# libmir/mir-optim

Measured on AMD Instinct MI355X. Metric: LM iterations/sec, higher is better.
Workload: dtype f64

## Files before the change

include/mir_optim_amd.h:

```cpp
#ifndef MIR_OPTIM_AMD_H
#define MIR_OPTIM_AMD_H

#include <stddef.h>
#include <stdint.h>

#ifdef __cplusplus
extern "C" {
#endif


typedef enum mir_least_squares_status {
    mir_ls_maxIterations = -1,
    mir_ls_furtherImprovement = 0,
    mir_ls_xConverged = 1,
    mir_ls_gConverged = 2,
    mir_ls_fConverged = 3,
    mir_ls_badBounds = -32,
    mir_ls_badGuess = -31,
    mir_ls_badMinStepQuality = -30,
    mir_ls_badGoodStepQuality = -29,
    mir_ls_badStepQuality = -28,
    mir_ls_badLambdaParams = -27,
    mir_ls_numericError = -26
} mir_least_squares_status;
// ... 29 lines not shown
    uint32_t maxIterations, maxAge;
    float jacobianEpsilon, absTolerance, relTolerance, gradTolerance, maxGoodResidual, maxStep,
          maxLambda, minLambda, minStepQuality, goodStepQuality, lambdaIncrease, lambdaDecrease;
    mir_box_qp_settings_s qpSettings;
} mir_least_squares_settings_s;

typedef struct mir_least_squares_result_d {
    int32_t status;
    uint32_t iterations, fCalls, gCalls;
    double residual;
    double lambda;
} mir_least_squares_result_d;
typedef struct mir_least_squares_result_s {
    int32_t status;
    uint32_t iterations, fCalls, gCalls;
    float residual, lambda;
} mir_least_squares_result_s;

typedef struct mir_slice_d { size_t length; double* ptr; } mir_slice_d;
typedef struct mir_slice_s { size_t length; float* ptr; } mir_slice_s;
typedef struct mir_slice_i { size_t length; int32_t* ptr; } mir_slice_i;

typedef void (*mir_least_squares_function_d)(void* context, size_t m, size_t n, const double* x, double* y);
typedef void (*mir_least_squares_jacobian_d)(void* context, size_t m, size_t n, const double* x, double* J);
typedef void (*mir_least_squares_function_s)(void* context, size_t m, size_t n, const float* x, float* y);
typedef void (*mir_least_squares_jacobian_s)(void* context, size_t m, size_t n, const float* x, float* J);

typedef struct mir_least_squares_task { void* context; void* function; } mir_least_squares_task;
typedef void (*mir_least_squares_task_function)(mir_least_squares_task task, uint32_t totalThreads,
                                                uint32_t threadId, uint32_t i);
typedef void (*mir_least_squares_thread_manager)(void* context, uint32_t count,
                                                 mir_least_squares_task taskContext,
                                                 mir_least_squares_task_function task);

size_t mir_least_squares_work_length(size_t m, size_t n);
size_t mir_least_squares_iwork_length(size_t m, size_t n);
size_t mir_box_qp_work_length(size_t n);
size_t mir_box_qp_iwork_length(size_t n);
size_t mir_box_qp_iwork_length_ilp64(size_t n);
size_t mir_least_squares_iwork_length_ilp64(size_t m, size_t n);
const char* mir_least_squares_status_string(mir_least_squares_status st);
void mir_least_squares_init_d(mir_least_squares_settings_d* settings);
void mir_least_squares_init_s(mir_least_squares_settings_s* settings);
void mir_least_squares_reset_d(mir_least_squares_settings_d* settings);
void mir_least_squares_reset_s(mir_least_squares_settings_s* settings);

mir_least_squares_result_d mir_optimize_least_squares_d(
    const mir_least_squares_settings_d* settings, size_t m, size_t n,
    double* x, const double* l, const double* u,
    mir_slice_d work, mir_slice_i iwork,
    void* fContext, mir_least_squares_function_d f,
    void* gContext, mir_least_squares_jacobian_d g,
    void* tmContext, mir_least_squares_thread_manager tm);

mir_least_squares_result_s mir_optimize_least_squares_s(
    const mir_least_squares_settings_s* settings, size_t m, size_t n,
    float* x, const float* l, const float* u,
    mir_slice_s work, mir_slice_i iwork,
    void* fContext, mir_least_squares_function_s f,
    void* gContext, mir_least_squares_jacobian_s g,
    void* tmContext, mir_least_squares_thread_manager tm);


typedef struct mir_lsq_comm mir_lsq_comm;
typedef struct mir_lsq_workspace mir_lsq_workspace;

typedef void (*mir_lsq_batched_function_d)(void* context, size_t m, size_t n, size_t p, const double* X, double* Y);
typedef void (*mir_lsq_batched_function_s)(void* context, size_t m, size_t n, size_t p, const float* X, float* Y);
enum {
    MIR_LSQ_DEVICE_CALLBACKS = 1u,
    MIR_LSQ_TIME_KERNELS = 2u,
    MIR_LSQ_FD_BASE_POINT = 4u
};

enum {
    MIR_LSQ_VARIANT_BROYDEN_REWRITE = 1u << 0,
    MIR_LSQ_VARIANT_FD_SEPARATE_FILL = 1u << 1,
    MIR_LSQ_VARIANT_NO_SPECULATION = 1u << 4,
    MIR_LSQ_VARIANT_NO_NULL_SKIP = 1u << 5,
    MIR_LSQ_VARIANT_SOLVE_BOUNDED = 1u << 6,
    MIR_LSQ_VARIANT_SOLVE_GENERIC = 1u << 10,
    MIR_LSQ_VARIANT_SOLVE_ONE_WORKGROUP = 1u << 11,
    MIR_LSQ_VARIANT_NO_FD_BASE_POINT = 1u << 14,
    MIR_LSQ_VARIANT_FD_HOST_COLUMNS = 1u << 13,
    MIR_LSQ_VARIANT_NO_PIPELINE = 1u << 22,
    MIR_LSQ_VARIANT_DEBUG_HELPERS_ABSENT = 1u << 12,
    MIR_LSQ_VARIANT_DEBUG_SOLVE = 1u << 7,
    MIR_LSQ_VARIANT_HOST_PROFILE = 1u << 8,
    MIR_LSQ_VARIANT_LR_CAP_SHIFT = 16
};

typedef struct mir_lsq_stats {
    uint64_t passes, accepted, rejected, step_guard_rejects;
    uint64_t jacobian_full, jacobian_broyden;
    uint64_t jtj_launches;
    uint64_t jtj_broyden_launches;
    double jtj_ms;
    double jtj_broyden_ms;
    double solve_ms;
    uint64_t solve_launches;
    double fd_ms;
    double total_ms;
    uint64_t qp_active_set_passes;
    uint64_t broyden_lr_columns;
    double jtj_fd_ms;
    uint64_t jtj_fd_launches;
    uint64_t elided_evaluations;
    uint64_t allreduce_calls[3];
    uint64_t allreduce_elems[3];
    uint64_t broyden_flushes;
    uint64_t jtj_resyncs;
    double fd_callback_ms;
    uint64_t fd_callback_calls, fd_callback_points;
    double trial_callback_ms;
    uint64_t trial_callback_calls, trial_callback_points;
    uint64_t library_launches;
    uint64_t round_launches[3];
    uint64_t rounds[3];
    double fd_host_wall_ms, fd_host_f_ms;
    uint64_t fd_host_columns;
    double host_f_ms;
    uint64_t host_f_calls;
    uint64_t fused_rounds;
    uint64_t fused_passes;
    uint64_t coop_timeouts;
} mir_lsq_stats;

typedef struct mir_lsq_trace_record {
    int32_t event;
    uint32_t iterations;
    double lambda, residual, trial_residual, dx_dot;
} mir_lsq_trace_record;
typedef struct mir_lsq_trace {
    mir_lsq_trace_record* records;
    uint64_t capacity;
    uint64_t count;
} mir_lsq_trace;

typedef struct mir_lsq_gpu_options {
    uint32_t struct_size;
    uint32_t flags;
    void* stream;
    mir_lsq_comm* comm;
    mir_lsq_workspace* workspace;
    void* fbContext;
    void* fb;
    uint32_t fd_batch;
    uint32_t variant;
    mir_lsq_stats* stats;
    mir_lsq_trace* trace;
    void* fbRowMajor;
    void* fbRowMajorDiff;
    uint32_t stats_size;
    uint32_t reserved0;
} mir_lsq_gpu_options;

mir_least_squares_result_d mir_optimize_least_squares_gpu_d(
    const mir_least_squares_settings_d* settings, size_t m, size_t n,
    double* x, const double* l, const double* u, const mir_lsq_gpu_options* options,
    void* fContext, mir_least_squares_function_d f,
    void* gContext, mir_least_squares_jacobian_d g,
    void* tmContext, mir_least_squares_thread_manager tm);
mir_least_squares_result_s mir_optimize_least_squares_gpu_s(
    const mir_least_squares_settings_s* settings, size_t m, size_t n,
    float* x, const float* l, const float* u, const mir_lsq_gpu_options* options,
    void* fContext, mir_least_squares_function_s f,
// ... 112 lines not shown
                                              const double* t, size_t t_stride, const double* data,
                                              mir_least_squares_result_d* results, const mir_lsq_batched_options* options,
                                              const mir_lsq_batched_extras* extras);
int mir_lsq_batched16_kernel_ex_d(const mir_least_squares_settings_d* settings, size_t count, size_t m, int model,
                                  double* x, const double* lower, const double* upper,
                                  const double* t, size_t t_stride, const double* data,
                                  mir_least_squares_result_d* results, const mir_lsq_batched_options* options,
                                  const mir_lsq_batched_extras* extras);
int mir_lsq_batched16_covariance_d(const mir_least_squares_settings_d* settings, size_t count, size_t m, int model,
                                   const double* x, const double* lower, const double* upper,
                                   const double* t, size_t t_stride, const double* data,
                                   const mir_least_squares_result_d* results, const mir_lsq_batched_options* options,
                                   const mir_lsq_batched_extras* extras);
int mir_lsq_batched16_jtj_d(size_t count, size_t m, size_t n, const double* J, const double* y, double* JJ, double* Jy, void* stream);

enum { MIR_LSQ_RESIDENT_NO_NULL_SKIP = 1u,
       MIR_LSQ_RESIDENT_UNBOUNDED = 2u,
       MIR_LSQ_RESIDENT_NO_LOOKAHEAD = 4u,
       MIR_LSQ_RESIDENT_DEBUG_DROP_WORKGROUP = 16u,
       MIR_LSQ_RESIDENT_ANALYTIC_JACOBIAN = 32u,
       MIR_LSQ_RESIDENT_NO_STAMPS = 8u           };
typedef struct mir_lsq_resident_stats {
    uint64_t rounds, passes, accepted, rejected, step_guard_rejects, jacobian_full, jacobian_broyden, qp_active_set_passes,
        elided_evaluations;
    uint64_t t_total, t_stage, t_worker, t_group, t_total_wait, t_solver, t_solve_body, t_cmd_wait;
    uint64_t t_w_eval, t_w_fd, t_w_prod;
    uint64_t t_w_mma;
    uint64_t lookahead_rejections;
    uint64_t t_look;
    uint64_t t_unpack, t_publish;
    uint32_t abort_code, grid, rows, groups;
} mir_lsq_resident_stats;
typedef struct mir_lsq_resident_options {
    uint32_t struct_size;
    uint32_t variant;
    void* stream;
    void* workspace;
    size_t workspace_bytes;
    mir_lsq_trace_record* trace_records;
    uint32_t trace_capacity;
    uint32_t max_workgroups;
    uint32_t* trace_count;
    mir_lsq_resident_stats* stats;
} mir_lsq_resident_options;

int mir_lsq_batched_posvx_s(size_t count, size_t n, const float* P, const float* rhs, float* x, int* info, void* stream);
int mir_lsq_batched_posvx_d(size_t count, size_t n, const double* P, const double* rhs, double* x, int* info, void* stream);
int mir_lsq_batched_posvx16_s(size_t count, size_t n, const float* P, const float* rhs, float* x, int* info, void* stream);
int mir_lsq_batched_posvx16_d(size_t count, size_t n, const double* P, const double* rhs, double* x, int* info, void* stream);

int mir_lsq_jtj_d(size_t m, size_t n, double* J, const double* y, const double* y_old, const double* dx,
                  int broyden, double* JJ, double* Jy, void* stream, float* kernel_ms);
int mir_lsq_jtj_s(size_t m, size_t n, float* J, const float* y, const float* y_old, const float* dx,
                  int broyden, float* JJ, float* Jy, void* stream, float* kernel_ms);
int mir_lsq_fd_jtj_d(size_t m, size_t n, const double* Yrm, const double* twh, const double* y, double* J,
                     double* JJ, double* Jy, void* stream, float* kernel_ms);
int mir_lsq_fd_diff_jtj_d(size_t m, size_t n, const double* Drm, const double* twh, const double* y, double* J,
                          double* JJ, double* Jy, void* stream, float* kernel_ms);
int mir_lsq_jtj_plan(size_t elem_size, size_t m, size_t n, int num_cu, int op, int aligned16, size_t out[10]);

enum { MIR_LSQ_LM_SOLVE_CHECK_GRAD = 1u, MIR_LSQ_LM_SOLVE_LAMBDA_FROM_STATE = 2u, MIR_LSQ_LM_SOLVE_FORCE_BOUNDED = 4u,
       MIR_LSQ_LM_SOLVE_GENERIC = 8u, MIR_LSQ_LM_SOLVE_ONE_WORKGROUP = 16u };
#define MIR_LSQ_LM_SOLVE_SENTINEL (-123456.0)
typedef struct { double lambda, new_dx_dot, predicted, trial_xnorm; int32_t qp_status, qp_iterations, flags, reserved; } mir_lsq_lm_solve_record_d;
typedef struct { float  lambda, new_dx_dot, predicted, trial_xnorm; int32_t qp_status, qp_iterations, flags, reserved; } mir_lsq_lm_solve_record_s;
int mir_lsq_lm_solve_d(const mir_least_squares_settings_d* settings, size_t n, double* JJ, double* Jy, double* x, double* lower,
                       double* upper, int ks, const double* lam, double state_lambda, unsigned mode, mir_lsq_lm_solve_record_d* rec,
                       double* dx, double* trial, double* jy_inf, int info[6]);
int mir_lsq_lm_solve_s(const mir_least_squares_settings_s* settings, size_t n, float* JJ, float* Jy, float* x, float* lower,
                       float* upper, int ks, const float* lam, float state_lambda, unsigned mode, mir_lsq_lm_solve_record_s* rec,
                       float* dx, float* trial, float* jy_inf, int info[6]);
int mir_lsq_lm_solve_class(size_t elem_size, size_t n, int bounded, int generic, int diagnostic, int out[3]);

int mir_lsq_lr_pass_d(size_t m, size_t n, int k, const double* J, double* U, double* D, const double* dx, const double* dx_dot,
                      const double* y, int count, const double* y_old, double* JJ, double* Jy, const mir_lsq_lm_solve_record_d* spec,
                      double absTolerance, double relTolerance, double* partials, double* reduced, double* sums, double* jy_inf,
                      int info[6]);
int mir_lsq_lr_pass_s(size_t m, size_t n, int k, const float* J, float* U, float* D, const float* dx, const float* dx_dot,
                      const float* y, int count, const float* y_old, float* JJ, float* Jy, const mir_lsq_lm_solve_record_s* spec,
                      float absTolerance, float relTolerance, float* partials, float* reduced, float* sums, float* jy_inf,
                      int info[6]);
int mir_lsq_lr_flush_d(size_t m, size_t n, int k, double* J, const double* U, const double* D, int info[2]);
int mir_lsq_lr_flush_s(size_t m, size_t n, int k, float* J, const float* U, const float* D, int info[2]);
int mir_lsq_lr_class(size_t elem_size, size_t n, int aligned, int out[2]);
int mir_lsq_lr_blocks(size_t m, int num_cu);

typedef struct {
    double lambda, mu, residual, trial_residual, dx_dot, new_dx_dot, predicted, trial_xnorm, jy_inf, improvement, rho, pad0;
    int32_t qp_status, qp_iterations, flags, decision; uint32_t iterations; int32_t accepted_k;
    uint32_t consumed, fcalls, rejects, guards, qp_active, null_tail, seq, coop_rescued; int32_t spec_ok;
} mir_lsq_lm_state_d;
typedef struct {
    float lambda, mu, residual, trial_residual, dx_dot, new_dx_dot, predicted, trial_xnorm, jy_inf, improvement, rho, pad0;
    int32_t qp_status, qp_iterations, flags, decision; uint32_t iterations; int32_t accepted_k;
    uint32_t consumed, fcalls, rejects, guards, qp_active, null_tail, seq, coop_rescued; int32_t spec_ok;
} mir_lsq_lm_state_s;
enum { MIR_LSQ_DECIDE_CHECK_GRAD = 1u, MIR_LSQ_DECIDE_LAMBDA_FROM_STATE = 2u, MIR_LSQ_DECIDE_SPEC_STATIC = 4u, MIR_LSQ_DECIDE_MIRROR = 8u };
int mir_lsq_decide_d(const mir_least_squares_settings_d* settings, size_t n, int ks, unsigned mode, uint32_t maxIterations, uint32_t seq,
                     mir_lsq_lm_state_d* state, mir_lsq_lm_solve_record_d* rec, double* sums, double* x, double* trial, double* dx_chain,
                     double* dx_acc, double* partials, int nparts, int pstride, mir_lsq_lm_state_d* host_state, double* host_x, int info[2]);
int mir_lsq_decide_s(const mir_least_squares_settings_s* settings, size_t n, int ks, unsigned mode, uint32_t maxIterations, uint32_t seq,
                     mir_lsq_lm_state_s* state, mir_lsq_lm_solve_record_s* rec, float* sums, float* x, float* trial, float* dx_chain,
                     float* dx_acc, float* partials, int nparts, int pstride, mir_lsq_lm_state_s* host_state, float* host_x, int info[2]);
int mir_lsq_fd_points_d(size_t n, const double* x, const double* lower, const double* upper, double eps, int with_base, double* X,
                        double* twh, double* twh_host, int info[2]);
int mir_lsq_fd_points_s(size_t n, const float* x, const float* lower, const float* upper, float eps, int with_base, float* X,
                        float* twh, float* twh_host, int info[2]);
int mir_lsq_fd_fill_d(size_t m, size_t n, size_t ldy, int j0, int pc, const double* Y, const double* twh, double* J, int col, int info[2]);
int mir_lsq_fd_fill_s(size_t m, size_t n, size_t ldy, int j0, int pc, const float* Y, const float* twh, float* J, int col, int info[2]);
int mir_lsq_entry_state_d(size_t m, const double* v, uint32_t seq, double* partials, double* sum, mir_lsq_lm_state_d* state,
                          mir_lsq_lm_state_d* host_state, double* partials2, double* sums2, mir_lsq_lm_state_d* st2, int info[3]);
int mir_lsq_entry_state_s(size_t m, const float* v, uint32_t seq, float* partials, float* sum, mir_lsq_lm_state_s* state,
                          mir_lsq_lm_state_s* host_state, float* partials2, float* sums2, mir_lsq_lm_state_s* st2, int info[3]);
int mir_lsq_sumsq_blocks(size_t m);
int mir_lsq_unpack_grad_d(size_t n, const double* packed, mir_lsq_lm_state_d* state, double* JJ, double* Jy, int info[2]);
int mir_lsq_unpack_grad_s(size_t n, const float* packed, mir_lsq_lm_state_s* state, float* JJ, float* Jy, int info[2]);

enum { MIR_LSQ_COVARIANCE_ABSOLUTE_SIGMA = 1u };
int mir_lsq_covariance_gpu_d(const mir_least_squares_settings_d* settings, size_t m, size_t n,
    const double* x, const double* l, const double* u, const mir_lsq_gpu_options* options,
    void* fContext, mir_least_squares_function_d f, void* gContext, mir_least_squares_jacobian_d g,
    void* tmContext, mir_least_squares_thread_manager tm,
    uint32_t flags, double* cov, double* residual_out, int* info);
int mir_lsq_covariance_gpu_s(const mir_least_squares_settings_s* settings, size_t m, size_t n,
    const float* x, const float* l, const float* u, const mir_lsq_gpu_options* options,
    void* fContext, mir_least_squares_function_s f, void* gContext, mir_least_squares_jacobian_s g,
    void* tmContext, mir_least_squares_thread_manager tm,
    uint32_t flags, float* cov, float* residual_out, int* info);
int mir_lsq_spd_inverse_d(size_t n, const double* P, const unsigned char* fixed, double* X, int* info, void* stream);
int mir_lsq_spd_inverse_s(size_t n, const float*  P, const unsigned char* fixed, float*  X, int* info, void* stream);
size_t mir_lsq_spd_inverse_work_bytes(size_t n, size_t elem_size);
int mir_lsq_spd_inverse_work_d(size_t n, const double* P, const unsigned char* fixed, double* X, int* info, void* work,
                               size_t work_bytes, void* stream);
int mir_lsq_spd_inverse_work_s(size_t n, const float* P, const unsigned char* fixed, float* X, int* info, void* work,
                               size_t work_bytes, void* stream);

mir_lsq_workspace* mir_lsq_workspace_create(size_t m, size_t n, size_t elem_size);
void mir_lsq_workspace_destroy(mir_lsq_workspace* ws);

int mir_lsq_rccl_unique_id(void* out_128_bytes);
mir_lsq_comm* mir_lsq_comm_create_rccl(int nranks, int rank, const void* unique_id_128_bytes);
typedef void (*mir_lsq_allreduce_fn)(void* ctx, double* device_buf, size_t count, void* stream);
mir_lsq_comm* mir_lsq_comm_create_callback(int nranks, int rank, mir_lsq_allreduce_fn fn, void* ctx);
int mir_lsq_comm_create_local_group(int nranks, mir_lsq_comm** out_comms);
void mir_lsq_comm_destroy(mir_lsq_comm* comm);
int mir_lsq_comm_record(mir_lsq_comm* comm, double* host_buf, size_t capacity);
size_t mir_lsq_comm_recorded(const mir_lsq_comm* comm);
mir_lsq_comm* mir_lsq_comm_create_replay(int nranks, int rank, const double* totals_host, size_t len, mir_lsq_comm* inner);
int mir_lsq_comm_replay_rewind(mir_lsq_comm* comm);
int mir_lsq_comm_replay_set_delay(mir_lsq_comm* comm, unsigned microseconds);
int mir_lsq_comm_ranks(const mir_lsq_comm* comm);
int mir_lsq_comm_describe(const mir_lsq_comm* comm, char* buf, size_t len);
int mir_lsq_comm_allreduce_d(mir_lsq_comm* comm, double* buf, size_t count, void* stream);
int mir_lsq_comm_allreduce_s(mir_lsq_comm* comm, float* buf, size_t count, void* stream);

int mir_lsq_device_count(void);
void* mir_lsq_device_malloc(size_t bytes);
void mir_lsq_device_free(void* p);
int mir_lsq_memcpy_h2d(void* dst_device, const void* src_host, size_t bytes, void* stream);
int mir_lsq_memcpy_d2h(void* dst_host, const void* src_device, size_t bytes, void* stream);
int mir_lsq_memcpy_d2d(void* dst_device, const void* src_device, size_t bytes, void* stream);

int mir_lsq_selftest_reductions(int rounds, int mismatches[4]);
void* mir_lsq_stream_create(void);
void mir_lsq_stream_destroy(void* stream);
int mir_lsq_stream_synchronize(void* stream);
// ... 43 lines not shown
```

mir_optim_amd/api.py:

```python
import ctypes as C
import enum
import os
import types

import numpy as np

from . import build as _build

__all__ = [
    "LeastSquaresStatus", "BoxQPStatus", "LeastSquaresSettings", "LeastSquaresResult", "BoxQPSettings",
    "LeastSquaresException", "optimize", "optimizeLeastSquares", "solveBoxQP", "leastSquaresStatusString",
    "mir_least_squares_work_length", "mir_least_squares_iwork_length", "mir_box_qp_work_length",
    "mir_box_qp_iwork_length", "GpuOptions", "Stats", "lib", "workloads_lib", "device_count",
    "DeviceBuffer", "Stream", "jtj", "fd_jtj", "DEVICE_CALLBACKS", "TIME_KERNELS", "optimizeLeastSquaresBatched", "batchedPosvx", "BATCHED_NO_LADDER", "BATCHED_DEVICE_BOUNDS",
    "solveBoxQPBatched", "BOX_QP_UNCONSTRAINED_SOLUTION",
    "MODEL_EXP_DECAY", "MODEL_EXP3_AFFINE", "MODEL_EXP_DECAY_PAD8", "MODEL16_EXP_HARM16", "MODEL16_GAUSS3_AFFINE", "batched16JtJ", "optimizeLeastSquaresBatched16", "ResultS", "Trace", "TraceRecord", "Spline", "FitSplineResult", "fitSpline",
    "fit_spline_residuals", "variant_lr_cap",
    "VARIANT_BROYDEN_REWRITE", "VARIANT_FD_SEPARATE_FILL", "VARIANT_NO_SPECULATION", "VARIANT_NO_NULL_SKIP",
    "VARIANT_SOLVE_BOUNDED", "VARIANT_DEBUG_SOLVE", "VARIANT_HOST_PROFILE", "VARIANT_SOLVE_GENERIC", "VARIANT_SOLVE_ONE_WORKGROUP", "VARIANT_DEBUG_HELPERS_ABSENT", "VARIANT_FD_HOST_COLUMNS",
    "VARIANT_NO_PIPELINE", "FD_BASE_POINT", "VARIANT_NO_FD_BASE_POINT", "BatchedOptions", "BatchedExtras", "BATCHED_ABSOLUTE_SIGMA", "BATCHED_BOUNDS_PER_PROBLEM",
    "covariance", "spdInverse", "COVARIANCE_ABSOLUTE_SIGMA",
    "fitSplineGpu", "splineEvalGpu", "fit_spline_eval_gpu", "fit_spline_eval_host", "fit_spline_factor",
    "lmSolve", "lm_solve_class",
    "lrPass", "lrFlush", "lr_class", "lr_blocks", "lr_len",
    "lm_state_dtype", "lmDecide", "fdPoints", "fdFill", "entryState", "sumsq_blocks", "unpackGrad",
]

MODEL_EXP_DECAY = 0
MODEL_EXP3_AFFINE = 1
MODEL_EXP_DECAY_PAD8 = 2
MODEL16_EXP_HARM16 = 16
MODEL16_GAUSS3_AFFINE = 17
_MODELS16 = (MODEL16_EXP_HARM16, MODEL16_GAUSS3_AFFINE)

DEVICE_CALLBACKS = 1
TIME_KERNELS = 2
FD_BASE_POINT = 4

VARIANT_BROYDEN_REWRITE = 1 << 0
VARIANT_FD_SEPARATE_FILL = 1 << 1
VARIANT_NO_SPECULATION = 1 << 4
VARIANT_NO_NULL_SKIP = 1 << 5
VARIANT_SOLVE_BOUNDED = 1 << 6
VARIANT_DEBUG_SOLVE = 1 << 7
VARIANT_HOST_PROFILE = 1 << 8
VARIANT_SOLVE_GENERIC = 1 << 10
VARIANT_SOLVE_ONE_WORKGROUP = 1 << 11
VARIANT_DEBUG_HELPERS_ABSENT = 1 << 12
VARIANT_FD_HOST_COLUMNS = 1 << 13
VARIANT_NO_FD_BASE_POINT = 1 << 14
VARIANT_NO_PIPELINE = 1 << 22


def variant_lr_cap(k):
    return (int(k) & 31) << 16


class LeastSquaresStatus(enum.IntEnum):
    maxIterations = -1
    furtherImprovement = 0
    xConverged = 1
    gConverged = 2
    fConverged = 3
    badBounds = -32
    badGuess = -31
    badMinStepQuality = -30
    badGoodStepQuality = -29
    badStepQuality = -28
    badLambdaParams = -27
    numericError = -26


class BoxQPStatus(enum.IntEnum):
    solved = 0
    numericError = 1
    maxIterations = 2


class LeastSquaresException(Exception):

    def __init__(self, status, result=None):
        self.status = LeastSquaresStatus(status)
        self.result = result
        super().__init__("mir-optim Least Squares: " + leastSquaresStatusString(status))


class _QPd(C.Structure):
    _fields_ = [("relTolerance", C.c_double), ("absTolerance", C.c_double), ("maxIterations", C.c_uint32)]


class _QPs(C.Structure):
    _fields_ = [("relTolerance", C.c_float), ("absTolerance", C.c_float), ("maxIterations", C.c_uint32)]


_FIELDS = ["jacobianEpsilon", "absTolerance", "relTolerance", "gradTolerance", "maxGoodResidual", "maxStep",
           "maxLambda", "minLambda", "minStepQuality", "goodStepQuality", "lambdaIncrease", "lambdaDecrease"]


class _Sd(C.Structure):
    _fields_ = ([("maxIterations", C.c_uint32), ("maxAge", C.c_uint32)] + [(k, C.c_double) for k in _FIELDS]
                + [("qpSettings", _QPd)])


class _Ss(C.Structure):
    _fields_ = ([("maxIterations", C.c_uint32), ("maxAge", C.c_uint32)] + [(k, C.c_float) for k in _FIELDS]
                + [("qpSettings", _QPs)])


class _Rd(C.Structure):
    _fields_ = [("status", C.c_int32), ("iterations", C.c_uint32), ("fCalls", C.c_uint32), ("gCalls", C.c_uint32),
                ("residual", C.c_double), ("lambda_", C.c_double)]


class _Rs(C.Structure):
    _fields_ = [("status", C.c_int32), ("iterations", C.c_uint32), ("fCalls", C.c_uint32), ("gCalls", C.c_uint32),
                ("residual", C.c_float), ("lambda_", C.c_float)]


ResultS = _Rs


class _SliceD(C.Structure):
    _fields_ = [("length", C.c_size_t), ("ptr", C.c_void_p)]


class _Task(C.Structure):
    _fields_ = [("context", C.c_void_p), ("function", C.c_void_p)]


class Stats(C.Structure):
    _fields_ = [("passes", C.c_uint64), ("accepted", C.c_uint64), ("rejected", C.c_uint64),
                ("step_guard_rejects", C.c_uint64), ("jacobian_full", C.c_uint64), ("jacobian_broyden", C.c_uint64),
                ("jtj_launches", C.c_uint64), ("jtj_broyden_launches", C.c_uint64), ("jtj_ms", C.c_double),
# ... 96 lines not shown

def lib():
    global _lib
    if _lib is None:
        L = _load(_build.SOLVER_LIB)
        sz = C.c_size_t
        for name in ("mir_least_squares_work_length", "mir_least_squares_iwork_length"):
            getattr(L, name).restype = sz
            getattr(L, name).argtypes = [sz, sz]
        for name in ("mir_box_qp_work_length", "mir_box_qp_iwork_length"):
            getattr(L, name).restype = sz
            getattr(L, name).argtypes = [sz]
        L.mir_box_qp_iwork_length_ilp64.restype = sz
        L.mir_box_qp_iwork_length_ilp64.argtypes = [sz]
        L.mir_least_squares_iwork_length_ilp64.restype = sz
        L.mir_least_squares_iwork_length_ilp64.argtypes = [sz, sz]
        L.mir_least_squares_status_string.restype = C.c_char_p
        L.mir_least_squares_status_string.argtypes = [C.c_int]
        for suf, S, R in (("d", _Sd, _Rd), ("s", _Ss, _Rs)):
            getattr(L, "mir_least_squares_init_" + suf).argtypes = [C.POINTER(S)]
            getattr(L, "mir_least_squares_reset_" + suf).argtypes = [C.POINTER(S)]
            fn = getattr(L, "mir_optimize_least_squares_" + suf)
            fn.restype = R
            fn.argtypes = [C.POINTER(S), sz, sz, C.c_void_p, C.c_void_p, C.c_void_p, _SliceD, _SliceD,
                           C.c_void_p, C.c_void_p, C.c_void_p, C.c_void_p, C.c_void_p, C.c_void_p]
            fn = getattr(L, "mir_optimize_least_squares_gpu_" + suf)
            fn.restype = R
            fn.argtypes = [C.POINTER(S), sz, sz, C.c_void_p, C.c_void_p, C.c_void_p, C.POINTER(GpuOptions),
                           C.c_void_p, C.c_void_p, C.c_void_p, C.c_void_p, C.c_void_p, C.c_void_p]
            fn = getattr(L, "mir_solve_box_qp_gpu_" + suf)
            fn.restype = C.c_int
            fn.argtypes = [C.c_void_p, sz, C.c_void_p, C.c_void_p, C.c_void_p, C.c_void_p, C.c_void_p, C.c_int,
                           C.POINTER(C.c_int)]
            fn = getattr(L, "mir_lsq_jtj_" + suf)
            fn.restype = C.c_int
            fn.argtypes = [sz, sz, C.c_void_p, C.c_void_p, C.c_void_p, C.c_void_p, C.c_int, C.c_void_p, C.c_void_p,
                           C.c_void_p, C.POINTER(C.c_float)]
            fn = getattr(L, "mir_lsq_covariance_gpu_" + suf)
            fn.restype = C.c_int
            fn.argtypes = [C.POINTER(S), sz, sz, C.c_void_p, C.c_void_p, C.c_void_p, C.POINTER(GpuOptions),
                           C.c_void_p, C.c_void_p, C.c_void_p, C.c_void_p, C.c_void_p, C.c_void_p,
                           C.c_uint32, C.c_void_p, C.c_void_p, C.POINTER(C.c_int)]
            fn = getattr(L, "mir_lsq_spd_inverse_" + suf)
            fn.restype = C.c_int
            fn.argtypes = [sz, C.c_void_p, C.c_void_p, C.c_void_p, C.c_void_p, C.c_void_p]
            fn = getattr(L, "mir_lsq_spd_inverse_work_" + suf)
            fn.restype = C.c_int
            fn.argtypes = [sz, C.c_void_p, C.c_void_p, C.c_void_p, C.c_void_p, C.c_void_p, sz, C.c_void_p]
        L.mir_lsq_spd_inverse_work_bytes.restype = sz
        L.mir_lsq_spd_inverse_work_bytes.argtypes = [sz, sz]
        L.mir_lsq_comm_create_local_group.restype = C.c_int
        L.mir_lsq_comm_create_local_group.argtypes = [C.c_int, C.POINTER(C.c_void_p)]
        L.mir_lsq_fd_diff_jtj_d.restype = C.c_int
        L.mir_lsq_fd_diff_jtj_d.argtypes = [sz, sz, C.c_void_p, C.c_void_p, C.c_void_p, C.c_void_p, C.c_void_p, C.c_void_p,
                                            C.c_void_p, C.POINTER(C.c_float)]
        L.mir_lsq_fd_jtj_d.restype = C.c_int
        L.mir_lsq_fd_jtj_d.argtypes = [sz, sz, C.c_void_p, C.c_void_p, C.c_void_p, C.c_void_p, C.c_void_p, C.c_void_p,
                                       C.c_void_p, C.c_void_p]
        L.mir_optimize_least_squares_batched_s.restype = C.c_int
        L.mir_optimize_least_squares_batched_s.argtypes = [C.POINTER(_Ss), sz, sz, C.c_int, C.c_void_p, C.c_void_p, C.c_void_p,
                                                           C.c_void_p, sz, C.c_void_p, C.c_void_p, C.POINTER(BatchedOptions)]
        L.mir_lsq_batched_kernel_s.restype = C.c_int
        L.mir_lsq_batched_kernel_s.argtypes = [C.POINTER(_Ss), sz, sz, C.c_int, C.c_void_p, C.c_void_p, C.c_void_p,
                                               C.c_void_p, sz, C.c_void_p, C.c_void_p, C.POINTER(BatchedOptions)]
        L.mir_lsq_jtj_plan.restype = C.c_int
        L.mir_lsq_jtj_plan.argtypes = [sz, sz, sz, C.c_int, C.c_int, C.c_int, C.POINTER(sz * 10)]
        L.mir_lsq_selftest_reductions.restype = C.c_int
        L.mir_lsq_selftest_reductions.argtypes = [C.c_int, C.POINTER(C.c_int * 4)]
        for suf, S, ct in (("d", _Sd, C.c_double), ("s", _Ss, C.c_float)):
            fn = getattr(L, "mir_lsq_lm_solve_" + suf)
            fn.restype = C.c_int
            fn.argtypes = [C.POINTER(S), sz, C.c_void_p, C.c_void_p, C.c_void_p, C.c_void_p, C.c_void_p, C.c_int, C.c_void_p, ct,
                           C.c_uint, C.c_void_p, C.c_void_p, C.c_void_p, C.c_void_p, C.POINTER(C.c_int * 6)]
        L.mir_lsq_lm_solve_class.restype = C.c_int
        L.mir_lsq_lm_solve_class.argtypes = [sz, sz, C.c_int, C.c_int, C.c_int, C.POINTER(C.c_int * 3)]
        for suf, ct in (("d", C.c_double), ("s", C.c_float)):
            fn = getattr(L, "mir_lsq_lr_pass_" + suf)
            fn.restype = C.c_int
            fn.argtypes = [sz, sz, C.c_int] + [C.c_void_p] * 6 + [C.c_int] + [C.c_void_p] * 4 + [ct, ct] + [C.c_void_p] * 4 \
                + [C.POINTER(C.c_int * 6)]
            fn = getattr(L, "mir_lsq_lr_flush_" + suf)
            fn.restype = C.c_int
            fn.argtypes = [sz, sz, C.c_int, C.c_void_p, C.c_void_p, C.c_void_p, C.POINTER(C.c_int * 2)]
        L.mir_lsq_lr_class.restype = C.c_int
        L.mir_lsq_lr_class.argtypes = [sz, sz, C.c_int, C.POINTER(C.c_int * 2)]
        L.mir_lsq_lr_blocks.restype = C.c_int
        L.mir_lsq_lr_blocks.argtypes = [sz, C.c_int]
        vp, i2 = C.c_void_p, C.POINTER(C.c_int * 2)
        for suf, S, ct in (("d", _Sd, C.c_double), ("s", _Ss, C.c_float)):
            for name, args in (("decide", [C.POINTER(S), sz, C.c_int, C.c_uint, C.c_uint32, C.c_uint32] + [vp] * 8 + [C.c_int, C.c_int, vp, vp, i2]),
                               ("fd_points", [sz, vp, vp, vp, ct, C.c_int, vp, vp, vp, i2]),
                               ("fd_fill", [sz, sz, sz, C.c_int, C.c_int, vp, vp, vp, C.c_int, i2]),
                               ("entry_state", [sz, vp, C.c_uint32] + [vp] * 7 + [C.POINTER(C.c_int * 3)]),
                               ("unpack_grad", [sz, vp, vp, vp, vp, i2])):
                fn = getattr(L, "mir_lsq_%s_%s" % (name, suf))
                fn.restype, fn.argtypes = C.c_int, args
        L.mir_lsq_sumsq_blocks.restype = C.c_int
        L.mir_lsq_sumsq_blocks.argtypes = [sz]
        L.mir_lsq_batched_posvx_s.restype = C.c_int
        L.mir_lsq_batched_posvx_s.argtypes = [sz, sz, C.c_void_p, C.c_void_p, C.c_void_p, C.c_void_p, C.c_void_p]
        L.mir_optimize_least_squares_batched_d.restype = C.c_int
        L.mir_optimize_least_squares_batched_d.argtypes = [C.POINTER(_Sd), sz, sz, C.c_int, C.c_void_p, C.c_void_p, C.c_void_p,
                                                           C.c_void_p, sz, C.c_void_p, C.c_void_p, C.POINTER(BatchedOptions)]
        L.mir_lsq_batched_kernel_d.restype = C.c_int
        L.mir_lsq_batched_kernel_d.argtypes = [C.POINTER(_Sd), sz, sz, C.c_int, C.c_void_p, C.c_void_p, C.c_void_p,
                                               C.c_void_p, sz, C.c_void_p, C.c_void_p, C.POINTER(BatchedOptions)]
        L.mir_lsq_batched_posvx_d.restype = C.c_int
        L.mir_lsq_batched_posvx_d.argtypes = [sz, sz, C.c_void_p, C.c_void_p, C.c_void_p, C.c_void_p, C.c_void_p]
        for suf, S in (("s", _Ss), ("d", _Sd)):
            for name in ("mir_optimize_least_squares_batched_ex_", "mir_lsq_batched_kernel_ex_", "mir_lsq_batched_covariance_"):
                fn = getattr(L, name + suf)
                fn.restype = C.c_int
                fn.argtypes = [C.POINTER(S), sz, sz, C.c_int, C.c_void_p, C.c_void_p, C.c_void_p, C.c_void_p, sz, C.c_void_p,
                               C.c_void_p, C.POINTER(BatchedOptions), C.POINTER(BatchedExtras)]
        for name in ("mir_optimize_least_squares_batched16_d", "mir_lsq_batched16_kernel_d", "mir_optimize_least_squares_batched16_ex_d",
                     "mir_lsq_batched16_kernel_ex_d", "mir_lsq_batched16_covariance_d"):
            fn = getattr(L, name)
            fn.restype = C.c_int
            fn.argtypes = [C.POINTER(_Sd), sz, sz, C.c_int, C.c_void_p, C.c_void_p, C.c_void_p, C.c_void_p, sz, C.c_void_p,
                           C.c_void_p, C.POINTER(BatchedOptions), C.POINTER(BatchedExtras)]
        L.mir_lsq_batched16_jtj_d.restype = C.c_int
        L.mir_lsq_batched16_jtj_d.argtypes = [sz, sz, sz, C.c_void_p, C.c_void_p, C.c_void_p, C.c_void_p, C.c_void_p]
        for name in ("box_qp_s", "box_qp_d", "box_qp16_s", "box_qp16_d"):
            fn = getattr(L, "mir_lsq_batched_" + name)
            fn.restype = C.c_int
            fn.argtypes = [C.c_void_p, sz, sz, C.c_void_p, C.c_void_p, C.c_void_p, C.c_void_p, sz, C.c_void_p, C.c_void_p,
                           C.c_void_p, C.c_uint, C.c_void_p]
        for suf in ("s", "d"):
            fn = getattr(L, "mir_lsq_batched_posvx16_" + suf)
            fn.restype = C.c_int
            fn.argtypes = [sz, sz, C.c_void_p, C.c_void_p, C.c_void_p, C.c_void_p, C.c_void_p]
        L.mir_lsq_comm_describe.restype = C.c_int
        L.mir_lsq_comm_describe.argtypes = [C.c_void_p, C.c_char_p, C.c_size_t]
        L.mir_lsq_workspace_create.restype = C.c_void_p
        L.mir_lsq_workspace_create.argtypes = [sz, sz, sz]
        L.mir_lsq_workspace_destroy.argtypes = [C.c_void_p]
        L.mir_lsq_rccl_unique_id.restype = C.c_int
        L.mir_lsq_rccl_unique_id.argtypes = [C.c_void_p]
        L.mir_lsq_comm_create_rccl.restype = C.c_void_p
        L.mir_lsq_comm_create_rccl.argtypes = [C.c_int, C.c_int, C.c_void_p]
        L.mir_lsq_comm_create_callback.restype = C.c_void_p
        L.mir_lsq_comm_create_callback.argtypes = [C.c_int, C.c_int, ALLREDUCE_FN, C.c_void_p]
        L.mir_lsq_comm_destroy.argtypes = [C.c_void_p]
        L.mir_lsq_comm_record.restype = C.c_int
        L.mir_lsq_comm_record.argtypes = [C.c_void_p, C.c_void_p, sz]
        L.mir_lsq_comm_recorded.restype = sz
        L.mir_lsq_comm_recorded.argtypes = [C.c_void_p]
        L.mir_lsq_comm_create_replay.restype = C.c_void_p
        L.mir_lsq_comm_create_replay.argtypes = [C.c_int, C.c_int, C.c_void_p, sz, C.c_void_p]
        L.mir_lsq_comm_replay_rewind.restype = C.c_int
        L.mir_lsq_comm_replay_rewind.argtypes = [C.c_void_p]
        L.mir_lsq_comm_replay_set_delay.restype = C.c_int
        L.mir_lsq_comm_replay_set_delay.argtypes = [C.c_void_p, C.c_uint]
        L.mir_lsq_comm_ranks.restype = C.c_int
        L.mir_lsq_comm_ranks.argtypes = [C.c_void_p]
        for name in ("mir_lsq_comm_allreduce_d", "mir_lsq_comm_allreduce_s"):
            getattr(L, name).restype = C.c_int
            getattr(L, name).argtypes = [C.c_void_p, C.c_void_p, sz, C.c_void_p]
        L.mir_lsq_device_count.restype = C.c_int
        L.mir_lsq_device_malloc.restype = C.c_void_p
        L.mir_lsq_device_malloc.argtypes = [sz]
        L.mir_lsq_device_free.argtypes = [C.c_void_p]
        for name in ("mir_lsq_memcpy_h2d", "mir_lsq_memcpy_d2h", "mir_lsq_memcpy_d2d"):
            getattr(L, name).restype = C.c_int
            getattr(L, name).argtypes = [C.c_void_p, C.c_void_p, sz, C.c_void_p]
        L.mir_lsq_stream_create.restype = C.c_void_p
# ... 483 lines not shown
    fn = L.mir_solve_box_qp_gpu_d if dtype == np.float64 else L.mir_solve_box_qp_gpu_s
    st = fn(C.byref(settings), n, P.ctypes.data, q.ctypes.data, l.ctypes.data, u.ctypes.data, xo.ctypes.data,
            1 if unconstrainedSolution else 0, C.byref(it))
    return BoxQPStatus(st), xo, it.value


BOX_QP_UNCONSTRAINED_SOLUTION = 1

LM_SOLVE_KINDS = ("wave", "workgroup", "big")
LM_SOLVE_SENTINEL = -123456.0
LM_SOLVE_CHAIN = 8
LM_FLAG_DX_NAN, LM_FLAG_X_NAN, LM_FLAG_STEP_TOO_LONG, LM_FLAG_GRAD_SMALL, LM_FLAG_NULL_STEP, LM_FLAG_COOP_RESCUED = 1, 2, 4, 16, 32, 64


def lm_solve_class(elem_size, n, bounded, generic=False, diagnostic=False):
    out = (C.c_int * 3)()
    rc = lib().mir_lsq_lm_solve_class(elem_size, n, int(bool(bounded)), int(bool(generic)), int(bool(diagnostic)), C.byref(out))
    if rc != 0:
        raise ValueError(f"mir_lsq_lm_solve_class: {rc}")
    return LM_SOLVE_KINDS[out[0]], int(out[1]), bool(out[2])


def lm_solve_record_dtype(dtype):
    f = np.dtype(dtype)
    return np.dtype([("lambda", f), ("new_dx_dot", f), ("predicted", f), ("trial_xnorm", f), ("qp_status", np.int32),
                     ("qp_iterations", np.int32), ("flags", np.int32), ("reserved", np.int32)])


def lmSolve(JJ, Jy, x, lower, upper, lam, settings=None, dtype=np.float64, state_lambda=0.0, check_grad=False,
            lambda_from_state=False, force_bounded=False, generic=False, one_workgroup=False):
    JJ = np.array(JJ, dtype=dtype, order="C")
    n = JJ.shape[0]
    if JJ.shape != (n, n):
        raise ValueError(f"JJ: n x n, not {JJ.shape}")
    vecs = [np.array(v, dtype=dtype, order="C") for v in (Jy, x, lower, upper)]
    if any(v.shape != (n,) for v in vecs):
        raise ValueError(f"Jy, x, lower, upper: {n} values each")
    lam = np.array(lam, dtype=dtype, order="C").reshape(-1)
    ks = lam.size
    if not 1 <= ks <= LM_SOLVE_CHAIN:
        raise ValueError(f"lam: 1 .. {LM_SOLVE_CHAIN} values, not {ks}")
    if settings is None:
        settings = LeastSquaresSettings(dtype)
    rec = np.zeros(ks, dtype=lm_solve_record_dtype(dtype))
    dx = np.zeros((LM_SOLVE_CHAIN, n), dtype=dtype)
    trial = np.zeros((LM_SOLVE_CHAIN, n), dtype=dtype)
    jy_inf = np.zeros(1, dtype=dtype)
    info = (C.c_int * 6)()
    mode = (1 if check_grad else 0) | (2 if lambda_from_state else 0) | (4 if force_bounded else 0) | (8 if generic else 0) \
        | (16 if one_workgroup else 0)
    fn = lib().mir_lsq_lm_solve_d if dtype == np.float64 else lib().mir_lsq_lm_solve_s
    rc = fn(C.byref(settings), n, JJ.ctypes.data, *(v.ctypes.data for v in vecs), ks, lam.ctypes.data, float(state_lambda), mode,
            rec.ctypes.data, dx.ctypes.data, trial.ctypes.data, jy_inf.ctypes.data, C.byref(info))
    if rc != 0:
        raise RuntimeError(f"mir_lsq_lm_solve failed: {rc}")
    return {"rec": rec, "dx": dx, "trial": trial, "jy_inf": jy_inf[0], "cls": (LM_SOLVE_KINDS[info[0]], int(info[1]), bool(info[2])),
            "helpers": int(info[3]), "guard": int(info[4]), "bands": int(info[5]), "inputs": (JJ, *vecs)}


LR_MAX = 16
LR_MAX_N = 512
LR_MAX_BLOCKS = 1024


def lr_len(n):
    return 2 * n + 2 * LR_MAX + 3


def lr_class(elem_size, n, aligned=True):
    out = (C.c_int * 2)()
    rc = lib().mir_lsq_lr_class(elem_size, n, int(bool(aligned)), C.byref(out))
    if rc != 0:
        raise ValueError(f"mir_lsq_lr_class: {rc}")
    return int(out[0]), bool(out[1])


def lr_blocks(m, num_cu=0):
    rc = lib().mir_lsq_lr_blocks(m, num_cu)
    if rc < 1:
        raise ValueError(f"mir_lsq_lr_blocks: {rc}")
    return rc


def lrPass(m, n, k, J, U, D, dx, dx_dot, y, y_old, JJ, Jy, dtype=np.float64, count=1, spec=None, absTolerance=0.0, relTolerance=0.0):
    dtype = np.dtype(dtype)
    nblk, ln = lr_blocks(m), lr_len(n)
    partials, reduced = np.zeros((nblk, ln), dtype=dtype), np.zeros(ln, dtype=dtype)
    sums, jy_inf = np.zeros(count, dtype=dtype), np.zeros(1, dtype=dtype)
    rec = None
    if spec is not None:
        rec = np.zeros(1, dtype=lm_solve_record_dtype(dtype))
        for key, v in spec.items():
            rec[key] = v
    info = (C.c_int * 6)()
    fn = lib().mir_lsq_lr_pass_d if dtype == np.float64 else lib().mir_lsq_lr_pass_s
    rc = fn(m, n, k, J, U, D, dx, dx_dot, y, count, y_old, JJ, Jy, rec.ctypes.data if rec is not None else None,
            float(absTolerance), float(relTolerance), partials.ctypes.data, reduced.ctypes.data, sums.ctypes.data, jy_inf.ctypes.data,
            C.byref(info))
    if rc != 0:
        raise RuntimeError(f"mir_lsq_lr_pass failed: {rc}")
    if info[2] != nblk:
        raise RuntimeError(f"mir_lsq_lr_pass ran {info[2]} workgroups, mir_lsq_lr_blocks said {nblk}")
    return {"partials": partials, "reduced": reduced, "sums": sums, "jy_inf": jy_inf[0], "cls": (int(info[0]), bool(info[1])),
            "nblk": nblk, "guard": int(info[3]), "bands": int(info[4]), "touched": int(info[5])}


def lrFlush(m, n, k, J, U, D, dtype=np.float64):
    info = (C.c_int * 2)()
    fn = lib().mir_lsq_lr_flush_d if np.dtype(dtype) == np.float64 else lib().mir_lsq_lr_flush_s
    rc = fn(m, n, k, J, U, D, C.byref(info))
    if rc != 0:
        raise RuntimeError(f"mir_lsq_lr_flush failed: {rc}")
    return int(info[0]), bool(info[1])


LM_FLAG_TRIAL_NOT_FINITE = 8
LM_DECIDE_REJECT, LM_DECIDE_ACCEPT, LM_DECIDE_ACCEPT_NO_PREDICTION, LM_DECIDE_NUMERIC_ERROR, LM_DECIDE_GRAD_SMALL = 1, 2, 3, 4, 5
LM_STATE_FLOATS = ("lambda", "mu", "residual", "trial_residual", "dx_dot", "new_dx_dot", "predicted", "trial_xnorm", "jy_inf",
                   "improvement", "rho", "pad0")
LM_STATE_INTS = (("qp_status", np.int32), ("qp_iterations", np.int32), ("flags", np.int32), ("decision", np.int32),
                 ("iterations", np.uint32), ("accepted_k", np.int32), ("consumed", np.uint32), ("fcalls", np.uint32),
                 ("rejects", np.uint32), ("guards", np.uint32), ("qp_active", np.uint32), ("null_tail", np.uint32), ("seq", np.uint32),
                 ("coop_rescued", np.uint32), ("spec_ok", np.int32))


def lm_state_dtype(dtype):
    f = np.dtype(dtype)
    names = list(LM_STATE_FLOATS) + [k for k, _ in LM_STATE_INTS]
    formats = [f] * len(LM_STATE_FLOATS) + [t for _, t in LM_STATE_INTS]
    offsets = [i * f.itemsize for i in range(12)] + [12 * f.itemsize + 4 * i for i in range(len(LM_STATE_INTS))]
    size = 12 * f.itemsize + 4 * len(LM_STATE_INTS)
    return np.dtype({"names": names, "formats": formats, "offsets": offsets, "itemsize": -(-size // f.itemsize) * f.itemsize})


def lmDecide(state, rec, sums, x, trial, dx_chain, dx_acc, settings=None, dtype=np.float64, check_grad=False, lambda_from_state=False,
             spec_static=False, mirror=True, maxIterations=1000, seq=1, partials=None, nparts=0):
    dtype = np.dtype(dtype)
    state = np.array(state, dtype=lm_state_dtype(dtype)).reshape(1).copy()
    rec = np.array(rec, dtype=lm_solve_record_dtype(dtype)).reshape(-1).copy()
    ks = rec.size
    x, dx_acc = (np.array(v, dtype=dtype, order="C").reshape(-1) for v in (x, dx_acc))
    n = x.size
    sums = np.array(sums, dtype=dtype, order="C").reshape(-1)
    trial, dx_chain = (np.array(v, dtype=dtype, order="C") for v in (trial, dx_chain))
    if sums.shape != (ks,) or trial.shape != (ks, n) or dx_chain.shape != (ks, n) or dx_acc.shape != (n,):
        raise ValueError("lmDecide: sums ks, trial and dx_chain ks x n, x and dx_acc n values")
    pstride = 0
    if nparts:
        partials = np.array(partials, dtype=dtype, order="C")
        if partials.ndim != 2 or partials.shape[0] != ks:
            raise ValueError("lmDecide: partials ks x pstride")
        pstride = partials.shape[1]
    else:
        partials = None
    if settings is None:
        settings = LeastSquaresSettings(dtype.type)
    host_state = np.zeros(1, dtype=lm_state_dtype(dtype))
    host_x = np.zeros(n, dtype=dtype)
    info = (C.c_int * 2)()
    mode = (1 if check_grad else 0) | (2 if lambda_from_state else 0) | (4 if spec_static else 0) | (8 if mirror else 0)
    fn = lib().mir_lsq_decide_d if dtype == np.float64 else lib().mir_lsq_decide_s
    rc = fn(C.byref(settings), n, ks, mode, maxIterations, seq, state.ctypes.data, rec.ctypes.data, sums.ctypes.data, x.ctypes.data,
            trial.ctypes.data, dx_chain.ctypes.data, dx_acc.ctypes.data, partials.ctypes.data if partials is not None else None,
            nparts, pstride, host_state.ctypes.data, host_x.ctypes.data, C.byref(info))
    if rc != 0:
        raise RuntimeError(f"mir_lsq_decide failed: {rc}")
    return {"state": state, "rec": rec, "sums": sums, "x": x, "trial": trial, "dx_chain": dx_chain, "dx_acc": dx_acc,
            "partials": partials, "host_state": host_state, "host_x": host_x, "guard": int(info[0]), "bands": int(info[1])}


def fdPoints(x, lower, upper, eps, dtype=np.float64, with_base=False):
    dtype = np.dtype(dtype)
    x, lower, upper = (np.array(v, dtype=dtype, order="C").reshape(-1) for v in (x, lower, upper))
    n = x.size
    X = np.zeros((2 * n + (1 if with_base else 0), n), dtype=dtype)
    twh, twh_host = np.zeros(n, dtype=dtype), np.zeros(n, dtype=dtype)
    info = (C.c_int * 2)()
    fn = lib().mir_lsq_fd_points_d if dtype == np.float64 else lib().mir_lsq_fd_points_s
    rc = fn(n, x.ctypes.data, lower.ctypes.data, upper.ctypes.data, float(dtype.type(eps)), int(bool(with_base)), X.ctypes.data, twh.ctypes.data,
            twh_host.ctypes.data, C.byref(info))
    if rc != 0:
        raise RuntimeError(f"mir_lsq_fd_points failed: {rc}")
    return {"X": X, "twh": twh, "twh_host": twh_host, "guard": int(info[0]), "bands": int(info[1])}


def fdFill(Y, twh, J, j0, pc, dtype=np.float64, col=False):
    dtype = np.dtype(dtype)
    Y, twh, J = np.array(Y, dtype=dtype, order="C"), np.array(twh, dtype=dtype, order="C").reshape(-1), np.array(J, dtype=dtype, order="C")
    m, n = J.shape
    if Y.shape[0] != 2 * pc or Y.shape[1] < m or twh.size != n:
        raise ValueError("fdFill: Y 2 pc x ldy with ldy >= m, twh n values")
    info = (C.c_int * 2)()
    fn = lib().mir_lsq_fd_fill_d if dtype == np.float64 else lib().mir_lsq_fd_fill_s
    rc = fn(m, n, Y.shape[1], j0, pc, Y.ctypes.data, twh.ctypes.data, J.ctypes.data, int(bool(col)), C.byref(info))
    if rc != 0:
# ... 70 lines not shown
        raise ValueError(f"l, u: both {n} values or both {count} x {n}, not {l.shape} and {u.shape}")
    shared = l.ndim == 1
    Pp = np.zeros((count, W, W), dtype=dtype); Pp[:, :n, :n] = P
    qp = np.zeros((count, W), dtype=dtype); qp[:, :n] = q
    lp = np.zeros((W,) if shared else (count, W), dtype=dtype); lp[..., :n] = l
    up = np.zeros((W,) if shared else (count, W), dtype=dtype); up[..., :n] = u
    xp = np.zeros((count, W), dtype=dtype)
    if x is not None:
        x = np.asarray(x, dtype=dtype)
        if x.shape != (count, n):
            raise ValueError(f"x: {count} x {n}, not {x.shape}")
        xp[:, :n] = x
    elif unconstrainedSolution:
        raise ValueError("unconstrainedSolution=True needs x, the unconstrained minimisers")
    return count, n, Pp, qp, lp, up, (0 if shared else W), xp


def solveBoxQPBatched(P, q, l, u, x=None, settings=None, dtype=np.float64, unconstrainedSolution=False):
    n_in = np.shape(P)[1] if np.ndim(P) == 3 else 0
    if n_in > 16:
        raise ValueError(f"solveBoxQPBatched: n = {n_in} is above 16, the limit of the batched kernels")
    wide = n_in > 8
    pack = _box_qp_batched_pack16 if wide else _box_qp_batched_pack
    count, n, Pp, qp, lp, up, bound_stride, xp = pack(P, q, l, u, x, dtype, unconstrainedSolution)
    dtype = Pp.dtype.type
    suf = "s" if dtype == np.float32 else "d"
    if settings is None:
        settings = BoxQPSettings(dtype)
    if count == 0:
        return np.zeros(0, dtype=np.int32), np.zeros((0, n), dtype=dtype), np.zeros(0, dtype=np.int32)
    L = lib()
    bufs = [DeviceBuffer(a) for a in (Pp, qp, lp, up, xp)]
    dst = DeviceBuffer(nbytes=count * 4, dtype=np.int32, shape=(count,))
    dit = DeviceBuffer(nbytes=count * 4, dtype=np.int32, shape=(count,))
    st = Stream()
    name = ("mir_lsq_batched_box_qp16_" if wide else "mir_lsq_batched_box_qp_") + suf
    rc = getattr(L, name)(C.addressof(settings), count, n, bufs[0].ptr, bufs[1].ptr, bufs[2].ptr, bufs[3].ptr, bound_stride,
                          bufs[4].ptr, dst.ptr, dit.ptr, BOX_QP_UNCONSTRAINED_SOLUTION if unconstrainedSolution else 0, st.handle)
    if rc != 0:
        raise RuntimeError(f"{name} failed: {rc}")
    st.synchronize()
    out = dst.download().copy(), bufs[4].download()[:, :n].copy(), dit.download().copy()
    for b in bufs + [dst, dit]:
        b.free()
    return out


def jtj(J, y, y_old=None, dx=None, dtype=np.float64):
    L = lib()
    J = np.ascontiguousarray(J, dtype=dtype)
    m, n = J.shape
    dJ = DeviceBuffer(J)
    dy = DeviceBuffer(np.ascontiguousarray(y, dtype=dtype))
    broyden = dx is not None
    dyo = DeviceBuffer(np.ascontiguousarray(y_old if broyden else y, dtype=dtype))
    ddx = DeviceBuffer(np.ascontiguousarray(dx if broyden else np.zeros(n), dtype=dtype))
    dJJ = DeviceBuffer(nbytes=n * n * J.itemsize, dtype=dtype, shape=(n, n))
    dJy = DeviceBuffer(nbytes=n * J.itemsize, dtype=dtype, shape=(n,))
    ms = C.c_float(0)
    fn = L.mir_lsq_jtj_d if dtype == np.float64 else L.mir_lsq_jtj_s
    rc = fn(m, n, dJ.ptr, dy.ptr, dyo.ptr, ddx.ptr, 1 if broyden else 0, dJJ.ptr, dJy.ptr, None, C.byref(ms))
    if rc != 0:
        raise RuntimeError(f"mir_lsq_jtj failed: {rc}")
    out = dJJ.download(), dJy.download(), dJ.download(), ms.value
    for b in (dJ, dy, dyo, ddx, dJJ, dJy):
        b.free()
    return out


JTJ_OPS = ("plain", "rewrite", "fd", "fd_diff")
JTJ_FAMILIES = ("none", "stream", "fdp", "pc32", "ring8", "fdp8", "wide")


def jtj_plan(elem_size, m, n, num_cu, op, aligned=True):
    out = (C.c_size_t * 10)()
    rc = lib().mir_lsq_jtj_plan(elem_size, m, n, num_cu, JTJ_OPS.index(op), int(bool(aligned)), C.byref(out))
    if rc != 0:
        raise ValueError(f"mir_lsq_jtj_plan: {rc}")
    d = dict(zip(("family", "ncb", "flat", "grid", "jobs", "lds", "slabs", "slab_len", "reduce_ncb", "workspace_slab_elems"), map(int, out)))
    d["family"] = JTJ_FAMILIES[d["family"]]
    return d


def fd_jtj(Yrm, twh, y, diff=False):
    L = lib()
    Yrm = np.ascontiguousarray(Yrm, dtype=np.float64)
    m, n2 = Yrm.shape
    n = n2 if diff else n2 // 2
    dY = DeviceBuffer(Yrm)
    dt = DeviceBuffer(np.ascontiguousarray(twh, dtype=np.float64))
    dy = DeviceBuffer(np.ascontiguousarray(y, dtype=np.float64))
    dJ = DeviceBuffer(nbytes=m * n * 8, dtype=np.float64, shape=(m, n))
    dJJ = DeviceBuffer(nbytes=n * n * 8, dtype=np.float64, shape=(n, n))
    dJy = DeviceBuffer(nbytes=n * 8, dtype=np.float64, shape=(n,))
    ms = C.c_float(0)
    rc = (L.mir_lsq_fd_diff_jtj_d if diff else L.mir_lsq_fd_jtj_d)(m, n, dY.ptr, dt.ptr, dy.ptr, dJ.ptr, dJJ.ptr, dJy.ptr, None, C.byref(ms))
    if rc != 0:
        raise RuntimeError(f"mir_lsq_fd_jtj_d failed: {rc}")
    out = dJ.download(), dJJ.download(), dJy.download(), ms.value
    for b in (dY, dt, dy, dJ, dJJ, dJy):
        b.free()
    return out



class Spline:

    def __init__(self, x, values, dtype=np.float64):
        self.dtype = dtype
        self.x = np.ascontiguousarray(x, dtype=dtype)
        self.values = np.ascontiguousarray(values, dtype=dtype)
        self.derivatives = np.zeros_like(self.values)
        suf = "d" if dtype == np.float64 else "s"
        getattr(lib(), "mir_spline_c2_derivatives_" + suf)(self.x.size, self.x.ctypes.data, self.values.ctypes.data,
                                                         self.derivatives.ctypes.data)
        self._eval = getattr(lib(), "mir_spline_eval_" + suf)

    def withTwoDerivatives(self, t):
        out = np.zeros(3, dtype=self.dtype)
        self._eval(self.x.size, self.x.ctypes.data, self.values.ctypes.data, self.derivatives.ctypes.data, t, out.ctypes.data)
        return out

    def __call__(self, t):
        if np.ndim(t) == 0:
            return self.withTwoDerivatives(float(t))[0]
        return np.array([self.withTwoDerivatives(float(v))[0] for v in np.asarray(t).ravel()]).reshape(np.shape(t))


class FitSplineResult:

    def __init__(self, leastSquaresResult, spline):
        self.leastSquaresResult = leastSquaresResult
        self.spline = spline


def fit_spline_residuals(points, x, lambda_, splineY):
    points = np.ascontiguousarray(points, dtype=np.float64)
    x = np.ascontiguousarray(x, dtype=np.float64)
    v = np.ascontiguousarray(splineY, dtype=np.float64)
    m = points.shape[0] + (1 if lambda_ == 0 else 0)
    y = np.zeros(m)
    lib().mir_fit_spline_residuals_d(points.shape[0], points.ctypes.data, x.size, x.ctypes.data, lambda_, v.ctypes.data, m,
                                     y.ctypes.data)
    return y


def fitSpline(settings, points, x, l, u, lambda_=0.0, dtype=np.float64):
    L = lib()
    points = np.ascontiguousarray(points, dtype=dtype)
    x = np.ascontiguousarray(x, dtype=dtype)
    lo = np.ascontiguousarray(l, dtype=dtype)
    up = np.ascontiguousarray(u, dtype=dtype)
    if not lambda_ >= 0:
        raise ValueError("fitSpline: lambda has to be non-negative")
    y = np.zeros(x.size, dtype=dtype)
    d = np.zeros(x.size, dtype=dtype)
    dbl = dtype == np.float64
    raw = (_Rd if dbl else _Rs)()
    fn = L.mir_fit_spline_d if dbl else L.mir_fit_spline_s
    rc = fn(C.byref(settings) if settings is not None else None, points.shape[0], points.ctypes.data, x.size,
            x.ctypes.data, lo.ctypes.data, up.ctypes.data, lambda_, None, y.ctypes.data, d.ctypes.data, C.byref(raw))
    if rc == 1:
        raise Exception("fitSpline: points.length has to be greater or equal x.length when lambda is 0.0")
    if rc != 0:
        raise ValueError("fitSpline: bad argument")
    res = LeastSquaresResult(raw)
    if res.status < 0:
        raise LeastSquaresException(int(res.status), res)
    return FitSplineResult(res, Spline(x, y, dtype))



def fitSplineGpu(settings, points, x, l, u, lambda_=0.0, dtype=np.float64, stats=None, variant=0, stream=None):
    L = lib()
    x = np.ascontiguousarray(x, dtype=dtype)
    lo = np.ascontiguousarray(l, dtype=dtype)
    up = np.ascontiguousarray(u, dtype=dtype)
    if not lambda_ >= 0:
        raise ValueError("fitSpline: lambda has to be non-negative")
    own = not isinstance(points, DeviceBuffer)
    if own:
        points = np.ascontiguousarray(points, dtype=dtype)
# ... 105 lines not shown
```

mir_optim_amd/csrc/broyden_launch.h:

```cpp
#pragma once

#include "common.h"
#include "solve_types.h"

namespace mirlsq {

template <typename T>
struct LrArgs {
    const T* J;
    T* U;
    const T* D;
    const T* dx;
    const T* dx_dot;
    const T* y;
    const T* y_old;
    T* partials;
    size_t m;
    int n;
    int k;
    const ChainRec<T>* spec_rec;
    T absTolerance, relTolerance;
};

constexpr int kLrMaxBlocks = 1024;
inline int lr_blocks(size_t m, int num_cu)
{
    const size_t G = (m + 3) / 4;
    size_t want = (G + 4 * 8 - 1) / (4 * 8);
    size_t cap = (size_t)num_cu * 4;
    if (cap > (size_t)kLrMaxBlocks) cap = kLrMaxBlocks;
    if (want > cap) want = cap;
    return (int)(want ? want : 1);
}

struct LrClass { int ncp; bool vec; };
inline LrClass lr_class(int n, bool aligned)
{
    const int chunks = (n + 31) / 32;
    int ncp = 1;
    while (ncp < chunks) ncp *= 2;
    return {ncp, n % 2 == 0 && aligned};
}
template <typename T> inline LrClass lr_class_of(int n, const T* J)
{
    return lr_class(n, reinterpret_cast<uintptr_t>(J) % (2 * sizeof(T)) == 0);
}

template <typename T> hipError_t lr_sweep(const LrArgs<T>& a, int nblk, hipStream_t s);
template <typename T> hipError_t lr_reduce(const T* partials, int nblk, int n, T* out, hipStream_t s);
template <typename T> hipError_t lr_finish(const T* lr, T* D, const T* dx, int k, int n, T* JJ, T* Jy, LmState<T>* st, hipStream_t s);
template <typename T> hipError_t lr_sumsq(const T* v, size_t m, int count, size_t vstride, T* partials, int pstride, int nblk, hipStream_t s);
template <typename T> hipError_t lr_sumsq_final(const T* partials, int pstride, int nblk, int count, T* out, hipStream_t s);
template <typename T> hipError_t lr_flush(T* J, const T* U, const T* D, int k, size_t m, int n, int num_cu, hipStream_t s);

}
```

mir_optim_amd/csrc/broyden_lr.h:

```cpp
#pragma once

#include "broyden_launch.h"
#include "common.h"
#include "solve_types.h"

namespace mirlsq {


template <typename T> struct LrPair;
template <> struct LrPair<double> { using type = double2; };
template <> struct LrPair<float> { using type = float2; };



template <typename T>
__device__ __forceinline__ bool lr_spec_go(const ChainRec<T>& r, T absTolerance, T relTolerance)
{
    const T dxn = dsqrt(r.new_dx_dot);
    return r.qp_status == 0 && !(r.flags & (kFlagDxNaN | kFlagXNaN | kFlagStepTooLong | kFlagNullStep | kFlagGradSmall))
        && (dxn > absTolerance && r.trial_xnorm > dxn * relTolerance);
}

template <typename T>
__device__ __forceinline__ T lr_wave_sumsq(const T* __restrict__ y, size_t m, size_t gb, size_t ge, int q)
{
    T yy = 0;
    for (size_t g0 = gb; g0 < ge; g0 += 8) {
        T v[8];
#pragma unroll
        for (int e = 0; e < 8; ++e) {
            const size_t row = 4 * (g0 + e) + q;
            v[e] = (g0 + e < ge && row < m) ? y[row] : T(0);
        }
#pragma unroll
        for (int e = 0; e < 8; ++e)
            if (g0 + e < ge) yy = dfma(v[e], v[e], yy);
    }
    yy += wave_shfl_xor(yy, 16);
    yy += wave_shfl_xor(yy, 32);
    return yy;
}

template <typename T, int NCP, bool VEC>
__global__ __launch_bounds__(256, (NCP <= 4 ? 4 : 1)) void k_broyden_lr(const LrArgs<T> a)
{
    using P2 = typename LrPair<T>::type;
    __shared__ T red[4][lr_len(kLrMaxN)];
    __shared__ T coef[kLrMax];
    const int lane = threadIdx.x & 63, wave = threadIdx.x >> 6;
    const int q = lane >> 4, p = lane & 15;
    const int n = a.n, k = a.k;
    const size_t m = a.m;
    const size_t G = (m + 3) / 4;
    const size_t nw = (size_t)gridDim.x * 4, wid = (size_t)blockIdx.x * 4 + wave;
    const size_t per = (G + nw - 1) / nw;
    const size_t gb = wid * per;
    const size_t ge = gb + per < G ? gb + per : G;
    if (a.spec_rec && !lr_spec_go(a.spec_rec[0], a.absTolerance, a.relTolerance)) {
        const T yy = lr_wave_sumsq(a.y, m, gb, ge, q);
        if (q == 0 && p == 0) red[wave][0] = yy;
        __syncthreads();
        const int len = lr_len(n);
        T* out = a.partials + (size_t)blockIdx.x * len;
        for (int e = threadIdx.x; e < len; e += blockDim.x) out[e] = e == lr_yy(n) ? (red[0][0] + red[1][0]) + (red[2][0] + red[3][0]) : T(0);
        return;
    }

    for (int l = wave; l < k; l += 4) {
        T s = 0;
        for (int j = lane; j < n; j += kWave) s += a.D[(size_t)l * n + j] * a.dx[j];
        s = wave_sum(s);
        if (lane == 0) coef[l] = s;
    }
    T d0[NCP], d1[NCP];
    int coff[NCP];
    bool ok0[NCP], ok1[NCP];
#pragma unroll
    for (int c = 0; c < NCP; ++c) {
        const int col = 32 * c + 2 * p;
        ok0[c] = col < n;
        ok1[c] = col + 1 < n;
        coff[c] = ok0[c] ? col : 0;
        const T t0 = a.dx[ok0[c] ? col : 0], t1 = a.dx[ok1[c] ? col + 1 : 0];
        d0[c] = ok0[c] ? t0 : T(0);
        d1[c] = ok1[c] ? t1 : T(0);
    }
    __syncthreads();
    const bool own = p < k;
    const T cp = own ? coef[p] : T(0);
    const T* __restrict__ Up = a.U + (size_t)(own ? p : 0) * m;
    T* __restrict__ Uk = a.U + (size_t)k * m;
    const T nd = -(T(1) / *a.dx_dot);

    T va0[NCP], va1[NCP], ga0[NCP], ga1[NCP];
#pragma unroll
    for (int c = 0; c < NCP; ++c) { va0[c] = 0; va1[c] = 0; ga0[c] = 0; ga1[c] = 0; }
    T wl = 0, hl = 0, uu = 0, uy = 0, yy = 0;

    constexpr int UNR = NCP == 1 ? 4 : (NCP == 2 ? 2 : 1);
    for (size_t g0 = gb; g0 < ge; g0 += UNR) {
        T v0[UNR][NCP], v1[UNR][NCP], ynv[UNR], yov[UNR], ulv[UNR];
#pragma unroll
        for (int e = 0; e < UNR; ++e) {
            const size_t g = g0 + e < ge ? g0 + e : ge - 1;
            const size_t row = 4 * g + q;
            const size_t rr = row < m ? row : m - 1;
            const T* __restrict__ rp = a.J + rr * (size_t)n;
#pragma unroll
            for (int c = 0; c < NCP; ++c) {
                if constexpr (VEC) {
                    typedef T lr_v2 __attribute__((ext_vector_type(2)));
                    const lr_v2 t = __builtin_nontemporal_load(reinterpret_cast<const lr_v2*>(rp + coff[c]));
                    v0[e][c] = t.x;
                    v1[e][c] = t.y;
                } else {
                    v0[e][c] = rp[coff[c]];
                    v1[e][c] = rp[ok1[c] ? coff[c] + 1 : 0];
                }
            }
            ynv[e] = a.y[rr];
            yov[e] = a.y_old[rr];
            ulv[e] = own ? Up[rr] : T(0);
        }
#pragma unroll
        for (int e = 0; e < UNR; ++e) {
            if (g0 + e < ge) {
                const size_t row = 4 * (g0 + e) + q;
                const bool rok = row < m;
                T yn = ynv[e];
                const T yo = yov[e], ul = ulv[e];
                T s = ul * cp;
#pragma unroll
                for (int c = 0; c < NCP; ++c) s += v0[e][c] * d0[c] + v1[e][c] * d1[c];
                s = sum16(s);
                T u = nd * ((yo - yn) + s);
                if (!rok) { u = 0; yn = 0; }
                if (rok && p == 0) Uk[row] = u;
#pragma unroll
                for (int c = 0; c < NCP; ++c) {
                    va0[c] += v0[e][c] * u;
                    va1[c] += v1[e][c] * u;
                    ga0[c] += v0[e][c] * yn;
                    ga1[c] += v1[e][c] * yn;
                }
                wl += ul * u;
                hl += ul * yn;
                uu += u * u;
                uy += u * yn;
                yy = dfma(yn, yn, yy);
            }
        }
    }

    auto qsum = [](T v) { v += wave_shfl_xor(v, 16); v += wave_shfl_xor(v, 32); return v; };
#pragma unroll
    for (int c = 0; c < NCP; ++c) { va0[c] = qsum(va0[c]); va1[c] = qsum(va1[c]); ga0[c] = qsum(ga0[c]); ga1[c] = qsum(ga1[c]); }
    wl = qsum(wl); hl = qsum(hl); uu = qsum(uu); uy = qsum(uy); yy = qsum(yy);
    if (q == 0) {
#pragma unroll
        for (int c = 0; c < NCP; ++c) {
            if (ok0[c]) { red[wave][coff[c]] = va0[c]; red[wave][n + coff[c]] = ga0[c]; }
            if (ok1[c]) { red[wave][coff[c] + 1] = va1[c]; red[wave][n + coff[c] + 1] = ga1[c]; }
        }
        red[wave][2 * n + p] = wl;
        red[wave][2 * n + kLrMax + p] = hl;
        if (p == 0) { red[wave][2 * n + 2 * kLrMax] = uu; red[wave][2 * n + 2 * kLrMax + 1] = uy; red[wave][lr_yy(n)] = yy; }
    }
    __syncthreads();
    const int len = lr_len(n);
    T* out = a.partials + (size_t)blockIdx.x * len;
    for (int e = threadIdx.x; e < len; e += blockDim.x) out[e] = (red[0][e] + red[1][e]) + (red[2][e] + red[3][e]);
}

template <typename T>
__global__ __launch_bounds__(32 * kReduceRanges) void k_lr_reduce(const T* __restrict__ partials, int nparts, int len, T* __restrict__ out)
{
    __shared__ T part[kReduceRanges][33];
    const int es = threadIdx.x & 31, sp = threadIdx.x >> 5;
    const int e = blockIdx.x * 32 + es;
    T s = 0;
    if (e < len) {
        const int per = (nparts + kReduceRanges - 1) / kReduceRanges;
        const int b0 = sp * per, b1 = (b0 + per < nparts) ? b0 + per : nparts;
#pragma unroll 8
        for (int b = b0; b < b1; ++b) s += partials[(size_t)b * len + e];
    }
    part[sp][es] = s;
    __syncthreads();
    if (sp == 0 && e < len) {
        T tot = part[0][es];
#pragma unroll
        for (int r = 1; r < kReduceRanges; ++r) tot += part[r][es];
        out[e] = tot;
    }
}

template <typename T>
__device__ inline T lr_reduce_scalar(const T* __restrict__ partials, int nparts, T* part )
{
    if ((int)threadIdx.x < kReduceRanges) {
        const int per = (nparts + kReduceRanges - 1) / kReduceRanges;
        const int b0 = (int)threadIdx.x * per, b1 = (b0 + per < nparts) ? b0 + per : nparts;
        T s = 0;
#pragma unroll 8
        for (int b = b0; b < b1; ++b) s += partials[b];
        part[threadIdx.x] = s;
    }
    __syncthreads();
    T tot = part[0];
#pragma unroll
    for (int r = 1; r < kReduceRanges; ++r) tot += part[r];
    __syncthreads();
    return tot;
}

template <typename T>
__global__ __launch_bounds__(256) void k_lr_sumsq(const T* __restrict__ v0, size_t m, size_t vstride, T* __restrict__ partials0, int pstride)
{
    __shared__ T red[4];
    const int lane = threadIdx.x & 63, wave = threadIdx.x >> 6;
    const T* __restrict__ v = v0 + (size_t)blockIdx.y * vstride;
    const size_t G = (m + 3) / 4;
    const size_t nw = (size_t)gridDim.x * 4, wid = (size_t)blockIdx.x * 4 + wave;
    const size_t per = (G + nw - 1) / nw;
    const size_t gb = wid * per;
    const size_t ge = gb + per < G ? gb + per : G;
    const T yy = lr_wave_sumsq(v, m, gb, ge, lane >> 4);
    if (lane == 0) red[wave] = yy;
    __syncthreads();
    if (threadIdx.x == 0) partials0[(size_t)blockIdx.y * pstride + blockIdx.x] = (red[0] + red[1]) + (red[2] + red[3]);
}
template <typename T>
__global__ __launch_bounds__(256) void k_lr_sumsq_final(const T* __restrict__ partials0, int pstride, int nparts, T* __restrict__ out)
{
    __shared__ T part[kReduceRanges];
    const T tot = lr_reduce_scalar(partials0 + (size_t)blockIdx.x * pstride, nparts, part);
    if (threadIdx.x == 0) out[blockIdx.x] = tot;
}

template <typename T>
__global__ __launch_bounds__(256) void k_lr_finish(const T* __restrict__ lr, T* __restrict__ D, const T* __restrict__ dx,
                                                   int k, int n, T* __restrict__ JJ, T* __restrict__ Jy, LmState<T>* st)
{
    __shared__ T v[kLrMaxN];
    __shared__ T red[4];
    const T* __restrict__ w = lr + 2 * n;
    const T* __restrict__ h = w + kLrMax;
    const T uu = lr[2 * n + 2 * kLrMax], uy = lr[2 * n + 2 * kLrMax + 1];
    const int i = blockIdx.x;
    if (i < n) {
        for (int j = threadIdx.x; j < n; j += blockDim.x) {
            T s = lr[j];
            for (int l = 0; l < k; ++l) s = dfma(D[(size_t)l * n + j], w[l], s);
            v[j] = s;
        }
        __syncthreads();
        for (int j = threadIdx.x; j < n; j += blockDim.x) {
            const int r = i >= j ? i : j, c = i >= j ? j : i;
            JJ[(size_t)i * n + j] += lr_jj_term(v[r], v[c], dx[r], dx[c], uu);
        }
        return;
    }
    T mx = 0;
    for (int j = threadIdx.x; j < n; j += blockDim.x) {
        T s = lr[n + j];
        for (int l = 0; l < k; ++l) s = dfma(D[(size_t)l * n + j], h[l], s);
        s = dfma(dx[j], uy, s);
        Jy[j] = s;
        const T av = dabs(s);
        if (av > mx) mx = av;
        D[(size_t)k * n + j] = dx[j];
    }
    mx = wave_max(mx);
    if ((threadIdx.x & 63) == 0) red[threadIdx.x >> 6] = mx;
    __syncthreads();
    if (threadIdx.x == 0) {
        T r = red[0];
        for (int wv = 1; wv < (int)(blockDim.x >> 6); ++wv) r = red[wv] > r ? red[wv] : r;
        st->jy_inf = r;
    }
}

template <typename T, int NCP, bool VEC>
__global__ __launch_bounds__(256) void k_lr_flush(T* J, const T* __restrict__ U, const T* __restrict__ D,
                                                  int k, size_t m, int n)
{
    using P2 = typename LrPair<T>::type;
    extern __shared__ unsigned char lr_smem[];
    T* Ds = reinterpret_cast<T*>(lr_smem);
    for (int e = threadIdx.x; e < k * n; e += blockDim.x) Ds[e] = D[e];
    __syncthreads();
    const int lane = threadIdx.x & 63;
    const int q = lane >> 4, p = lane & 15;
    int coff[NCP];
    bool ok0[NCP], ok1[NCP];
#pragma unroll
    for (int c = 0; c < NCP; ++c) {
        const int col = 32 * c + 2 * p;
        ok0[c] = col < n;
        ok1[c] = col + 1 < n;
        coff[c] = ok0[c] ? col : 0;
    }
    const size_t G = (m + 3) / 4;
    const size_t wave_id = ((size_t)blockIdx.x * blockDim.x + threadIdx.x) >> 6;
    const size_t nwaves = ((size_t)gridDim.x * blockDim.x) >> 6;
    for (size_t g = wave_id; g < G; g += nwaves) {
        const size_t row = 4 * g + q;
        const bool rok = row < m;
        const size_t rr = rok ? row : m - 1;
        T* rp = J + rr * (size_t)n;
        const T* sp = rp;
        T v0[NCP], v1[NCP];
#pragma unroll
        for (int c = 0; c < NCP; ++c) {
            if constexpr (VEC) {
                typedef T lr_v2 __attribute__((ext_vector_type(2)));
                const lr_v2 t = __builtin_nontemporal_load(reinterpret_cast<const lr_v2*>(sp + coff[c]));
                v0[c] = t.x;
                v1[c] = t.y;
            } else {
                v0[c] = sp[coff[c]];
                v1[c] = sp[ok1[c] ? coff[c] + 1 : 0];
            }
        }
        for (int l = 0; l < k; ++l) {
            const T ul = U[(size_t)l * m + rr];
#pragma unroll
            for (int c = 0; c < NCP; ++c) {
                v0[c] += ul * Ds[l * n + coff[c]];
                v1[c] += ul * Ds[l * n + (ok1[c] ? coff[c] + 1 : 0)];
            }
        }
        if (rok) {
#pragma unroll
            for (int c = 0; c < NCP; ++c) {
                if constexpr (VEC) {
                    if (ok0[c]) {
                        typedef T lr_v2 __attribute__((ext_vector_type(2)));
                        lr_v2 t; t.x = v0[c]; t.y = v1[c];
                        __builtin_nontemporal_store(t, reinterpret_cast<lr_v2*>(rp + coff[c]));
                    }
                } else {
                    if (ok0[c]) rp[coff[c]] = v0[c];
                    if (ok1[c]) rp[coff[c] + 1] = v1[c];
                }
            }
        }
    }
}

}
```

mir_optim_amd/csrc/common.h:

```cpp
#pragma once

#include <hip/hip_runtime.h>

#include <cfloat>
#include <cmath>
#include <cstdint>
#include <cstdio>
#include <utility>

namespace mirlsq {

constexpr int kWave = 64;

#define MIRLSQ_HIP_CHECK(expr)                                                                  \
    do {                                                                                        \
        hipError_t _e = (expr);                                                                 \
        if (_e != hipSuccess) {                                                                 \
            std::fprintf(stderr, "[mir_optim_amd] HIP error %s at %s:%d: %s\n",                 \
                         hipGetErrorName(_e), __FILE__, __LINE__, #expr);                       \
            return _e;                                                                          \
        }                                                                                       \
    } while (0)

inline thread_local uint64_t tl_launches = 0;
#define MIRLSQ_LAUNCH(...) do { ++::mirlsq::tl_launches; hipLaunchKernelGGL(__VA_ARGS__); } while (0)

__device__ inline double dfma(double a, double b, double c) { return __builtin_fma(a, b, c); }
__device__ inline float dfma(float a, float b, float c) { return __builtin_fmaf(a, b, c); }
constexpr int kLrMax = 16;
__host__ __device__ constexpr int lr_len(int n) { return 2 * n + 2 * kLrMax + 3; }
__host__ __device__ constexpr int lr_yy(int n) { return 2 * n + 2 * kLrMax + 2; }
constexpr int kLrMaxN = 512;
constexpr int kReduceRanges = 32;
template <typename T>
__device__ __forceinline__ T lr_jj_term(T vr, T vc, T dr, T dc, T uu)
{
#pragma clang fp contract(off)
    return dfma(uu * dr, dc, dfma(vr, dc, dr * vc));
}

template <typename T> struct Lim;
template <> struct Lim<double> {
    static constexpr double eps = DBL_EPSILON, max = DBL_MAX, min_normal = DBL_MIN;
    __host__ __device__ static double inf() { return __builtin_huge_val(); }
};
template <> struct Lim<float> {
    static constexpr float eps = FLT_EPSILON, max = FLT_MAX, min_normal = FLT_MIN;
    __host__ __device__ static float inf() { return __builtin_huge_valf(); }
};

template <typename T> struct Mma;
template <> struct Mma<double> {
    using Acc = __attribute__((ext_vector_type(4))) double;
    __device__ static inline Acc mma(double a, double b, Acc c) {
        return __builtin_amdgcn_mfma_f64_16x16x4f64(a, b, c, 0, 0, 0);
    }
    __host__ __device__ static inline int row(int lane, int r) { return (lane >> 4) + 4 * r; }
    __host__ __device__ static constexpr int perm(int h) { return 4 * (h & 3) + (h >> 2); }
};
template <> struct Mma<float> {
    using Acc = __attribute__((ext_vector_type(4))) float;
    __device__ static inline Acc mma(float a, float b, Acc c) {
        return __builtin_amdgcn_mfma_f32_16x16x4f32(a, b, c, 0, 0, 0);
    }
    __host__ __device__ static inline int row(int lane, int r) { return 4 * (lane >> 4) + r; }
    __host__ __device__ static constexpr int perm(int h) { return h; }
};

template <typename T> __device__ inline T wave_shfl_xor(T v, int mask) { return __shfl_xor(v, mask, kWave); }

template <int N> __device__ inline int dpp_row_ror(int v)
{
    return __builtin_amdgcn_update_dpp(0, v, 0x120 + N, 0xF, 0xF, false);
}
template <int N> __device__ inline double dpp_row_ror(double v)
{
    const int lo = dpp_row_ror<N>(__double2loint(v));
    const int hi = dpp_row_ror<N>(__double2hiint(v));
    return __hiloint2double(hi, lo);
}
template <int N> __device__ inline float dpp_row_ror(float v)
{
    return __int_as_float(dpp_row_ror<N>(__float_as_int(v)));
}

template <int N> __device__ inline int dpp_row_bcast(int v)
{
    return __builtin_amdgcn_mov_dpp(v, 0x150 + N, 0xF, 0xF, true);
}
template <int N> __device__ inline double dpp_row_bcast(double v)
{
    const int lo = dpp_row_bcast<N>(__double2loint(v));
    const int hi = dpp_row_bcast<N>(__double2hiint(v));
    return __hiloint2double(hi, lo);
}
template <int N> __device__ inline float dpp_row_bcast(float v)
{
    return __int_as_float(dpp_row_bcast<N>(__float_as_int(v)));
}

__device__ inline void wave_lds_fence()
{
    __builtin_amdgcn_fence(__ATOMIC_RELEASE, "wavefront");
    asm volatile("" ::: "memory");
    __builtin_amdgcn_fence(__ATOMIC_ACQUIRE, "wavefront");
}

__device__ inline void lds_barrier()
{
    __builtin_amdgcn_fence(__ATOMIC_RELEASE, "workgroup", "local");
    __builtin_amdgcn_s_barrier();
// ... 138 lines not shown
```

mir_optim_amd/csrc/driver.h:

```cpp
#pragma once

#include <hip/hip_runtime.h>

#include <atomic>
#include <chrono>
#include <cmath>
#include <cstdlib>
#include <cstring>
#include <mutex>
#include <thread>
#include <vector>

#include "../../include/mir_optim_amd.h"
#include "broyden_launch.h"
#include "comm.h"
#include "common.h"
#include "jtj_plan.h"
#include "solve_launch.h"
#include "solve_types.h"

struct mir_lsq_workspace {
    size_t m = 0, n = 0, elem = 0;
    void* dev = nullptr;
    size_t dev_bytes = 0;
// ... 42 lines not shown
    using T = decltype(Settings::minStepQuality);
    if (!(0 <= S->minStepQuality && S->minStepQuality < 1)) return mir_ls_badMinStepQuality;
    if (!(0 <= S->goodStepQuality && S->goodStepQuality <= 1)) return mir_ls_badGoodStepQuality;
    if (!(S->minStepQuality < S->goodStepQuality)) return mir_ls_badStepQuality;
    if (!(1 <= S->lambdaIncrease && S->lambdaIncrease <= std::sqrt(Lim<T>::max))) return mir_ls_badLambdaParams;
    if (!(std::sqrt(Lim<T>::min_normal) <= S->lambdaDecrease && S->lambdaDecrease <= 1)) return mir_ls_badLambdaParams;
    return 0;
}

inline void cpu_relax()
{
#if defined(__x86_64__) || defined(__i386__)
    __builtin_ia32_pause();
#elif defined(__aarch64__)
    asm volatile("yield" ::: "memory");
#else
    std::atomic_signal_fence(std::memory_order_seq_cst);
#endif
}

bool device_available();
int query_num_cu();

template <typename T>
struct Buffers {
    T *J, *y, *mB, *ytmp;
    T *X, *twh;
    T *x, *lower, *upper, *dx, *dx_acc, *trial, *Jy, *JJ, *packed, *partials, *sum;
    LmState<T>* st;
    ChainRec<T>* rec;
    T* slabs;
    T *lrD, *lrvec, *lrpart;
    SolveScratch<T> sc[kChainMax];
    size_t bytes;
};

constexpr int kPartials = 1024;

inline int sumsq_blocks(size_t m)
{
    int nb = (int)((m + 4095) / 4096);
    if (nb > kPartials) nb = kPartials;
    return nb < 1 ? 1 : nb;
}

template <typename T>
inline void fd_widths(const T* x, const T* lower, const T* upper, T eps, size_t n, T* twh)
{
    for (size_t j = 0; j < n; ++j) {
        const T save = x[j];
        T xmh = save - eps, xph = save + eps;
        xmh = std::fmax(xmh, lower[j]);
        xph = std::fmin(xph, upper[j]);
        twh[j] = xph - xmh;
    }
}

template <typename T> Buffers<T> carve(void* base, size_t m, size_t n, int num_cu);
template <typename T> mir_lsq_workspace* workspace_create(size_t m, size_t n);
void workspace_destroy(mir_lsq_workspace* ws);

struct EventPair { hipEvent_t a, b; int kind; };

template <typename T>
struct Solver {
    using Settings = typename Abi<T>::Settings;
    using Result = typename Abi<T>::Result;
    using F = typename Abi<T>::F;
    using G = typename Abi<T>::G;
    using FB = typename Abi<T>::FB;

    const Settings* S;
    size_t m;
    uint32_t n;
    T* xh;
    const T *lh, *uh;
    void* fctx; F f;
    void* gctx; G g;
    void* tmctx; mir_least_squares_thread_manager tm;
    void* fbctx; FB fb;
    FB fbr = nullptr;
    FB fbd = nullptr;
    int fd_fused = 0;
    bool fd_base_point = false;
    bool fd_entry_ready = false;
    size_t fd_entry_event = (size_t)-1;
    uint64_t launches_early = 0;
    uint64_t launches_held = 0;
    int sums_pending = 0;
    uint32_t fd_batch;
    bool device_cb;
    bool time_kernels;
    mir_lsq_comm* comm;
    mir_lsq_stats* stats;
    mir_lsq_trace* trace = nullptr;

    hipStream_t stream = nullptr;
    bool own_stream = false;
    mir_lsq_workspace* ws = nullptr;
    bool own_ws = false;
    Buffers<T> B;
    JtjPlan plan;
    LmSettingsDev<T> sd;
    uint32_t variant = 0;
    bool dbg_solve = false, no_speculation = false, lowrank = true, no_null_skip = false, host_profile = false;
    mir_lsq_stats stats_local{};
    mir_lsq_stats* stats_user = nullptr;
    size_t stats_bytes = 0;
    uint64_t launches_mark = 0;
    int round_kind = -1;
    uint64_t launches_excluded = 0;
    std::atomic<uint64_t> worker_launches{0};
    int lr_cap = kLrMax;
    int lr_k = 0;
    int device = 0, caller_device = -1;
    T* y = nullptr;
    T* mB = nullptr;
    T* fr = nullptr;
    bool has_bounds = true;
    bool tail_null = false;
    bool fused = false;
    bool spec_enqueue = false;
    size_t spec_events_from = 0;
    bool big_solve = false;
    bool coop_disabled = false;

    LmState<T>* st_h;
    LmState<T>* st_slot[2] = {nullptr, nullptr};
    LmState<T>* st_slot_d[2] = {nullptr, nullptr};
    T* x_slot[2] = {nullptr, nullptr};
    T* x_slot_d[2] = {nullptr, nullptr};
    T* x_h = nullptr;
    uint32_t seq = 0;
    T* trial_h;
    std::vector<T> twh_h;
    std::vector<EventPair> events;
    Result ret;

    struct Slot { T* p = nullptr; T* yp = nullptr; T* ym = nullptr; };
    std::vector<Slot> slots;
    std::vector<int> slot_count;
    std::mutex fd_mutex;
    std::atomic<bool> fd_failed{false};
    bool fd_panel_mode = false;
    std::atomic<uint32_t> fd_streams_used{0};
    std::atomic<uint64_t> fd_f_ns{0};
    std::atomic<uint32_t> fd_tasks_run{0};

    double hp_ms[6] = {0, 0, 0, 0, 0, 0};
    struct HpScope {
        Solver* s; int cat; std::chrono::steady_clock::time_point t0;
        HpScope(Solver* s_, int c) : s(s_), cat(c) { if (s->host_profile) t0 = std::chrono::steady_clock::now(); }
        ~HpScope() {
            if (!s->host_profile) return;
            const double ms = std::chrono::duration<double, std::milli>(std::chrono::steady_clock::now() - t0).count();
            s->hp_ms[cat] += ms;
            if (ms > s->hp_ms[5]) s->hp_ms[5] = ms;
        }
    };

    bool ok(hipError_t e, const char* what)
    {
        if (e == hipSuccess) return true;
        std::fprintf(stderr, "[mir_optim_amd] %s failed: %s\n", what, hipGetErrorName(e));
        return false;
    }
// ... 70 lines not shown
```

mir_optim_amd/csrc/launch_broyden.hip:

```cpp
#include <hip/hip_runtime.h>

#include <type_traits>

#include "broyden_launch.h"
#include "launch_util.h"
#include "broyden_lr.h"

namespace mirlsq {

namespace {
template <typename F>
hipError_t lr_dispatch(LrClass c, F&& f)
{
#define MIRLSQ_LR_CASE(NCP)                                                                               \
    case NCP:                                                                                             \
        return c.vec ? f(std::integral_constant<int, NCP>{}, std::true_type{}) : f(std::integral_constant<int, NCP>{}, std::false_type{});
    switch (c.ncp) {
        MIRLSQ_LR_CASE(1)
        MIRLSQ_LR_CASE(2)
        MIRLSQ_LR_CASE(4)
        MIRLSQ_LR_CASE(8)
        MIRLSQ_LR_CASE(16)
    }
#undef MIRLSQ_LR_CASE
    return hipErrorInvalidValue;
}
}
template <typename T>
hipError_t lr_sweep(const LrArgs<T>& a, int nblk, hipStream_t s)
{
    if (a.n > kLrMaxN || a.k < 0 || a.k >= kLrMax) return hipErrorInvalidValue;
    return lr_dispatch(lr_class_of<T>(a.n, a.J), [&](auto ncp, auto vec) {
        MIRLSQ_LAUNCH((k_broyden_lr<T, decltype(ncp)::value, decltype(vec)::value>), dim3(nblk), dim3(256), 0, s, a);
        return hipGetLastError();
    });
}

template <typename T>
hipError_t lr_flush(T* J, const T* U, const T* D, int k, size_t m, int n, int num_cu, hipStream_t s)
{
    if (k <= 0) return hipSuccess;
    if (n > kLrMaxN || k > kLrMax) return hipErrorInvalidValue;
    const size_t G = (m + 3) / 4;
    size_t blocks = (G + 3) / 4;
    if (blocks > (size_t)num_cu * 8) blocks = (size_t)num_cu * 8;
    if (blocks < 1) blocks = 1;
    const size_t lds = (size_t)k * n * sizeof(T);
    return lr_dispatch(lr_class_of<T>(n, J), [&](auto ncp, auto vec) {
        MIRLSQ_LAUNCH((k_lr_flush<T, decltype(ncp)::value, decltype(vec)::value>), dim3((unsigned)blocks), dim3(256), lds, s, J, U, D, k, m, n);
        return hipGetLastError();
    });
}

template <typename T>
hipError_t lr_reduce(const T* partials, int nblk, int n, T* out, hipStream_t s)
{
    const int len = lr_len(n);
    MIRLSQ_LAUNCH(k_lr_reduce<T>, dim3((len + 31) / 32), dim3(32 * kReduceRanges), 0, s, partials, nblk, len, out);
    return hipGetLastError();
}

template <typename T>
hipError_t lr_finish(const T* lr, T* D, const T* dx, int k, int n, T* JJ, T* Jy, LmState<T>* st, hipStream_t s)
{
    MIRLSQ_LAUNCH(k_lr_finish<T>, dim3(n + 1), dim3(256), 0, s, lr, D, dx, k, n, JJ, Jy, st);
    return hipGetLastError();
}

template <typename T>
hipError_t lr_sumsq(const T* v, size_t m, int count, size_t vstride, T* partials, int pstride, int nblk, hipStream_t s)
{
    if (count < 1 || nblk < 1 || nblk > pstride) return hipErrorInvalidValue;
    MIRLSQ_LAUNCH(k_lr_sumsq<T>, dim3(nblk, count), dim3(256), 0, s, v, m, vstride, partials, pstride);
    return hipGetLastError();
}
template <typename T>
hipError_t lr_sumsq_final(const T* partials, int pstride, int nblk, int count, T* out, hipStream_t s)
{
    MIRLSQ_LAUNCH(k_lr_sumsq_final<T>, dim3(count), dim3(256), 0, s, partials, pstride, nblk, out);
    return hipGetLastError();
}

#define MIRLSQ_INSTANTIATE(T)                                                                                             \
    template hipError_t lr_sweep<T>(const LrArgs<T>&, int, hipStream_t);                                                  \
    template hipError_t lr_reduce<T>(const T*, int, int, T*, hipStream_t);                                                \
    template hipError_t lr_finish<T>(const T*, T*, const T*, int, int, T*, T*, LmState<T>*, hipStream_t);                 \
    template hipError_t lr_sumsq<T>(const T*, size_t, int, size_t, T*, int, int, hipStream_t);                            \
    template hipError_t lr_sumsq_final<T>(const T*, int, int, int, T*, hipStream_t);                                      \
    template hipError_t lr_flush<T>(T*, const T*, const T*, int, size_t, int, int, hipStream_t);
MIRLSQ_INSTANTIATE(double)
MIRLSQ_INSTANTIATE(float)
#undef MIRLSQ_INSTANTIATE

}

MIRLSQ_DEFINE_PRELOAD(broyden)
```

mir_optim_amd/csrc/solver_jacobian.hip:

```cpp
#include "driver.h"
#include "launch_util.h"
#include "misc_kernels.h"

namespace mirlsq {

template <typename T>
bool Solver<T>::broyden_lowrank(const T* y_dev, const T* yold_dev)
{
    T* U = static_cast<T*>(ws->ulr);
    if (lr_k >= lr_cap) {
        const uint64_t launches_before = launches_now();
        struct Excl { Solver* s; uint64_t l0; ~Excl() { s->launches_excluded += s->launches_now() - l0; } } excl{this, launches_before};
        if (!ok(lr_flush<T>(B.J, U, B.lrD, lr_k, m, (int)n, ws->num_cu, stream), "broyden flush")) return false;
        lr_k = 0;
        if (stats) stats->broyden_flushes++;
        if (!plain_products(yold_dev)) return false;
        if (stats) stats->jtj_resyncs++;
    }
    LrArgs<T> a{};
    a.J = B.J; a.U = U; a.D = B.lrD; a.dx = B.dx_acc; a.dx_dot = &B.st->dx_dot; a.y = y_dev; a.y_old = yold_dev;
    a.partials = B.lrpart; a.m = m; a.n = (int)n; a.k = lr_k;
    const int nblk = lr_blocks(m, ws->num_cu), len = lr_len((int)n);
    ev_begin(1);
    if (!ok(lr_sweep<T>(a, nblk, stream), "broyden sweep")) return false;
    ev_end();
    if (!ok(lr_reduce<T>(B.lrpart, nblk, (int)n, B.lrvec, stream), "broyden reduce")) return false;
    if (comm && !allreduce(B.lrvec, (size_t)len, 1)) return false;
    if (!ok(lr_finish<T>(B.lrvec, B.lrD, B.dx_acc, lr_k, (int)n, B.JJ, B.Jy, B.st, stream), "broyden finish")) return false;
    if (stats) stats->broyden_lr_columns += (uint64_t)lr_k;
    ++lr_k;
    return true;
}

template <typename T>
bool Solver<T>::plain_products(const T* y_vec)
{
    JtjArgs<T> a{};
    a.J = B.J; a.Jout = B.J; a.y = y_vec; a.y_old = y_vec; a.dx = B.dx_acc; a.dx_dot = &B.st->dx_dot;
    a.slabs = B.slabs; a.m = m; a.n = (int)n;
    const bool direct = unpack_in_reduce(JtjOp::plain);
    ev_begin(0);
    if (!ok(jtj_run<T>(plan, JtjOp::plain, a, B.packed, stream, direct ? unpack_target() : JtjUnpack<T>{}), "jtj kernel")) return false;
    ev_end();
    return finish_products(direct);
}

template <typename T>
bool Solver<T>::finish_products(bool direct)
{
    if (direct) return ok(hipGetLastError(), "jtj reduce");
    if (comm && !allreduce(B.packed, (size_t)n * (n + 1) / 2 + n, 0)) return false;
    return ok(jtj_unpack<T>(B.packed, (int)n, B.JJ, B.Jy, B.st, stream), "unpack");
}

template <typename T>
bool Solver<T>::jacobian_products(bool broyden, const T* y_dev, const T* yold_dev)
{
    if (broyden && lowrank) return broyden_lowrank(y_dev, yold_dev);
    if (!broyden) lr_k = 0;
    JtjArgs<T> a{};
    a.J = B.J; a.Jout = B.J; a.y = y_dev; a.y_old = yold_dev; a.dx = B.dx_acc; a.dx_dot = &B.st->dx_dot;
    a.slabs = B.slabs; a.m = m; a.n = (int)n;
    if (!broyden && fd_fused) {
        const JtjOp op = fd_fused == 2 ? JtjOp::fd_diff : JtjOp::fd;
        fd_fused = 0;
        a.J = static_cast<const T*>(ws->ypanel); a.twh = B.twh;
        const bool direct = unpack_in_reduce(op);
        ev_begin(3);
        if (!ok(jtj_run<T>(plan, op, a, B.packed, stream, direct ? unpack_target() : JtjUnpack<T>{}), "fd + jtj kernel")) return false;
        ev_end();
        return finish_products(direct);
    }
    const JtjOp op = broyden ? JtjOp::rewrite : JtjOp::plain;
    const bool direct = unpack_in_reduce(op);
    ev_begin(broyden ? 1 : 0);
    if (!ok(jtj_run<T>(plan, op, a, B.packed, stream, direct ? unpack_target() : JtjUnpack<T>{}), "jtj kernel")) return false;
    ev_end();
    return finish_products(direct);
}

template <typename T>
void Solver<T>::fd_widths_host()
{
    fd_widths<T>(xh, lh, uh, S->jacobianEpsilon, n, twh_h.data());
}

template <typename T>
bool Solver<T>::fd_panel(size_t& pb, bool& use_diff)
{
    pb = n;
    size_t cap = (size_t)64 << 30;
    if (ws->ypanel_bytes < 2 * pb * m * sizeof(T)) {
        size_t free_b = 0, total_b = 0;
        if (hipMemGetInfo(&free_b, &total_b) == hipSuccess) {
            const size_t have = ws->ypanel_bytes + free_b;
            if (have / 2 < cap) cap = have / 2;
        }
        if (cap < ((size_t)1 << 30)) cap = (size_t)1 << 30;
    }
    if (2 * pb * m * sizeof(T) > cap) {
        pb = cap / (2 * m * sizeof(T));
        if (pb >= 64) pb -= pb % 64;
    }
    if (pb < 1) pb = 1;
    if (fb && fd_batch && fd_batch / 2 < pb) pb = fd_batch / 2 ? fd_batch / 2 : 1;
    const bool no_fuse = (variant & MIR_LSQ_VARIANT_FD_SEPARATE_FILL) != 0;
    use_diff = fbd && plan.fd_diff.kernel != JtjKernel::none && pb == n && !no_fuse;
    const size_t need = use_diff ? (pb * m + (fd_base_point ? m : 0)) * sizeof(T) : 2 * pb * m * sizeof(T);
    if (ws->ypanel_bytes < need) {
        if (ws->ypanel) (void)hipFree(ws->ypanel);
        ws->ypanel = nullptr; ws->ypanel_bytes = 0;
        if (!ok(hipMalloc(&ws->ypanel, need), "hipMalloc(FD panel)")) return false;
        ws->ypanel_bytes = need;
    }
    return true;
}

template <typename T>
bool Solver<T>::fd_entry(bool& done)
{
    done = false;
    if (!fd_base_point || !device_cb || g || !fbd) return true;
    size_t pb;
    bool use_diff;
    if (!fd_panel(pb, use_diff)) return false;
    if (!use_diff) return true;
    MIRLSQ_LAUNCH(k_fd_points<T>, dim3(n + 1), dim3(64), 0, stream, B.x, B.lower, B.upper, sd.jacobianEpsilon, (int)n, B.X, B.twh);
    launches_early = 1;
    T* Y = static_cast<T*>(ws->ypanel);
    ev_begin(4);
    fd_entry_event = time_kernels ? events.size() - 1 : (size_t)-1;
    fbd(fbctx, m, n, 2 * (size_t)n + 1, B.X, Y);
    ev_end();
    if (!ok(hipMemcpyAsync(y, Y + m * (size_t)n, m * sizeof(T), hipMemcpyDeviceToDevice, stream), "D2D entry residual")) return false;
    fd_entry_ready = true;
    done = true;
    return ok(hipGetLastError(), "fd entry callback");
}
template <typename T>
void Solver<T>::fd_entry_discard()
{
    fd_entry_ready = false;
    launches_early = launches_held = 0;
    if (fd_entry_event < events.size()) events[fd_entry_event].kind = -1;
}

template <typename T>
bool Solver<T>::fd_device()
{
// ... 242 lines not shown
```

mir_optim_amd/csrc/solver_loop.hip:

```cpp
#include "driver.h"
#include "launch_util.h"
#include "misc_kernels.h"

namespace mirlsq {

template <typename T>
void Solver<T>::ev_begin(int kind)
{
    if (!time_kernels) return;
    HpScope hp(this, 0);
    EventPair p{};
    p.kind = spec_enqueue ? kind + 100 : kind;
    if (ws->event_pool.size() < 2 * (events.size() + 1)) {
        hipEvent_t ea, eb;
        (void)hipEventCreate(&ea);
        (void)hipEventCreate(&eb);
        ws->event_pool.push_back(ea);
        ws->event_pool.push_back(eb);
    }
    p.a = ws->event_pool[2 * events.size()];
    p.b = ws->event_pool[2 * events.size() + 1];
    (void)hipEventRecord(p.a, stream);
    events.push_back(p);
}
// ... 212 lines not shown
    if (vec_dev && !ok(hipMemcpyAsync(trial_h, vec_dev, n * sizeof(T), hipMemcpyDeviceToHost, stream), "D2H vec")) return false;
    return ok(hipStreamSynchronize(stream), "sync");
}

template <typename T>
void Solver<T>::print_solve_dbg(bool fused_round)
{
    long long h[32];
    if (hipMemcpy(h, B.sc[0].dbg, sizeof h, hipMemcpyDeviceToHost) != hipSuccess) return;
    if (fused_round)
        std::fprintf(stderr, "[solve dbg] fused round head (10ns ticks): decision + publication %lld (loads landed %lld, decided + point copied %lld, fence + sequence number %lld)  n x n side of the Broyden pass %lld\n", h[27] - h[26], h[29] - h[26], h[30] - h[29], h[31] - h[30], h[28] - h[27]);
    std::fprintf(stderr, "[solve dbg] (10ns ticks) build %lld  copy/equil %lld  scale %lld  potrf %lld  potrs %lld  refine %lld  epilogue %lld  total %lld  shader MHz %.0f  [matvec1 %lld berr %lld]\n",
                 h[1] - h[0], h[2] - h[1], h[3] - h[2], h[4] - h[3], h[5] - h[4], h[6] - h[5], h[8] - h[7], h[8] - h[0], (double)(h[10] - h[9]) / (double)(h[8] - h[0]) * 100.0, h[11] - h[5], h[12] - h[11]);
    if (n <= 128)
        std::fprintf(stderr, "[solve dbg] load (10ns ticks): kernel entry -> loads landed %lld (of which inside posvx %lld)  reduction + LDS commit %lld  rest of the phase %lld\n",
                     h[24] - h[0], h[24] - h[2], h[25] - h[24], h[3] - h[25]);
    if (n <= 128)
        std::fprintf(stderr, "[solve dbg] refinement (10ns ticks): residual 1 %lld  berr 1 %lld  potrs 2 %lld  residual 2 %lld  rest %lld  (correction applied: %lld)\n",
                     h[11] - h[5], h[12] - h[11], h[13] - h[12], h[14] - h[13], h[6] - h[14], h[15]);
    if (n <= 128)
        std::fprintf(stderr, "[solve dbg] lds_potrf, wave 0 (shader cycles, summed over the panels): diagonal update + factor %lld  wait %lld  rows below %lld  wait %lld\n", h[20], h[21], h[22], h[23]);
    if (n > 128)
        std::fprintf(stderr, "[solve dbg] potrf_panel steps (10ns ticks, summed over the panels): earlier panels on MFMA %lld (of which publishing / waiting for the helpers' look-ahead jobs %lld)  diagonal rows %lld  other rows + store %lld\n", h[16], h[19], h[17], h[18]);
}

template <typename T>
LmSolveArgs<T> Solver<T>::solve_args(int ks, const T* lam, bool check_grad, bool lambda_from_state)
{
    LmSolveArgs<T> a{};
    a.JJ = B.JJ; a.Jy = B.Jy; a.x = B.x; a.lower = B.lower; a.upper = B.upper;
    a.dx = B.dx; a.trial = B.trial; a.st = B.st; a.rec = B.rec; a.set = sd; a.n = (int)n;
    for (int k = 0; k < kChainMax; ++k) { a.sc[k] = B.sc[k]; a.lam[k] = (lam && k < ks) ? lam[k] : T(0); }
    a.f_in_lds = solve_nb((int)n, (int)sizeof(T)) > 0;
    a.check_grad = check_grad ? 1 : 0;
    a.lambda_from_state = lambda_from_state ? 1 : 0;
    if (!dbg_solve) a.sc[0].dbg = nullptr;
    a.coop_w = coop_width((int)n, ws->num_cu, big_solve && !(variant & MIR_LSQ_VARIANT_SOLVE_ONE_WORKGROUP) && !coop_disabled);
    a.coop_epoch = a.coop_w > 1 ? ++ws->solve_epoch : 0;
    a.coop_absent = (variant & MIR_LSQ_VARIANT_DEBUG_HELPERS_ABSENT) ? 1 : 0;
    return a;
}
template <typename T>
bool Solver<T>::enqueue_solve(int ks, const T* lam, bool check_grad, bool lambda_from_state)
{
    const LmSolveArgs<T> a = solve_args(ks, lam, check_grad, lambda_from_state);
    ev_begin(2);
    {
        HpScope hp(this, 4);
        if (!ok(launch_lm_solve<T>(a, ks, has_bounds, big_solve, stream), "solve launch")) return false;
    }
    ev_end();
    return true;
}

template <typename T>
DecideArgs<T> Solver<T>::decide_args(int ks, bool check_grad, bool lambda_from_state)
{
    DecideArgs<T> d{};
    d.sums = B.sum + 1; d.rec = B.rec; d.st = B.st; d.set = sd; d.x = B.x; d.trial = B.trial; d.dx_chain = B.dx;
    d.dx_acc = B.dx_acc; d.n = (int)n; d.ks = ks; d.check_grad = check_grad ? 1 : 0;
    d.lambda_from_state = lambda_from_state ? 1 : 0;
    ++seq;
    d.host_st = st_slot_d[seq & 1]; d.host_x = x_slot_d[seq & 1]; d.seq = seq;
    d.maxIterations = S->maxIterations;
    d.partials = B.partials; d.nparts = sums_pending; d.pstride = kPartials;
    sums_pending = 0;
    return d;
}
template <typename T>
bool Solver<T>::enqueue_decide(int ks, bool check_grad, bool lambda_from_state, const T* sum_v)
{
    if (sum_v && !trial_sums(sum_v, ks, m)) return false;
    const DecideArgs<T> d = decide_args(ks, check_grad, lambda_from_state);
    MIRLSQ_LAUNCH(k_decide_chain<T>, dim3(1), dim3(kSolveThreads), 0, stream, d);
    return ok(hipGetLastError(), "decide kernel");
}

template <typename T>
bool Solver<T>::enqueue_fused_tail(const T* ytr, bool check_grad, bool lambda_from_state)
{
    spec_events_from = events.size();
    if (stats) stats->fused_rounds++;
    LrArgs<T> a{};
    a.J = B.J; a.U = static_cast<T*>(ws->ulr); a.D = B.lrD; a.dx = B.dx; a.dx_dot = &B.rec[0].new_dx_dot; a.y = ytr; a.y_old = y;
    a.partials = B.lrpart; a.m = m; a.n = (int)n; a.k = lr_k;
    a.spec_rec = B.rec; a.absTolerance = sd.absTolerance; a.relTolerance = sd.relTolerance;
    const int nblk = lr_blocks(m, ws->num_cu), len = lr_len((int)n);
    spec_enqueue = true;
    ev_begin(1);
    const bool swept = ok(lr_sweep<T>(a, nblk, stream), "broyden sweep");
    ev_end();
    spec_enqueue = false;
    if (!swept || !ok(lr_reduce<T>(B.lrpart, nblk, (int)n, B.lrvec, stream), "broyden reduce")) return false;
    if (comm && !allreduce(B.lrvec, (size_t)len, 1)) return false;
    LmSolveArgs<T> sa = solve_args(1, nullptr, true, false);
    sa.lambda_from_device = 1;
    sa.fused = 1;
    sa.dec = decide_args(1, check_grad, lambda_from_state);
    sa.dec.sums = B.lrvec + lr_yy((int)n);
    sa.dec.spec_static = 1;
    sa.fin_lr = B.lrvec; sa.fin_D = B.lrD; sa.fin_JJ = B.JJ; sa.fin_Jy = B.Jy; sa.fin_k = lr_k;
    spec_enqueue = true;
    ev_begin(2);
    bool good;
    {
        HpScope hp(this, 4);
        good = ok(launch_lm_solve<T>(sa, 1, has_bounds, false, stream), "fused round launch");
    }
    ev_end();
    spec_enqueue = false;
    return good;
}
template <typename T>
void Solver<T>::commit_spec_round()
{
    for (size_t i = spec_events_from; i < events.size(); ++i) if (events[i].kind >= 100) events[i].kind -= 100;
    if (stats) {
        stats->jacobian_broyden++;
        stats->fused_passes++;
        stats->broyden_lr_columns += (uint64_t)lr_k;
    }
    ++lr_k;
}
template <typename T>
void Solver<T>::drop_spec_round()
{
    for (size_t i = spec_events_from; i < events.size(); ++i) if (events[i].kind >= 100) events[i].kind = -1;
}

template <typename T>
typename Solver<T>::Result Solver<T>::run()
{
    ret.status = mir_ls_numericError; ret.iterations = 0; ret.fCalls = 0; ret.gCalls = 0;
    ret.residual = Lim<T>::inf(); ret.lambda = 0;
    const auto t_start = std::chrono::steady_clock::now();
    launches_mark = launches_now();

    {
        bool finite = true;
        for (uint32_t i = 0; i < n; ++i) if (!(-Lim<T>::inf() < xh[i] && xh[i] < Lim<T>::inf())) finite = false;
        if (m == 0 || n == 0 || !finite) { ret.status = mir_ls_badGuess; return ret; }
        for (uint32_t i = 0; i < n; ++i) if (!(lh[i] <= xh[i]) || !(xh[i] <= uh[i])) { ret.status = mir_ls_badBounds; return ret; }
        if (const int bad = bad_settings(S)) { ret.status = bad; return ret; }
    }
    if (!device_available()) return ret;
    if (!setup()) { teardown(); return ret; }
    has_bounds = (variant & MIR_LSQ_VARIANT_SOLVE_BOUNDED) != 0;
    for (uint32_t i = 0; i < n; ++i)
        if (lh[i] > -Lim<T>::inf() || uh[i] < Lim<T>::inf()) has_bounds = true;

    const uint32_t maxAge = S->maxAge ? S->maxAge : (g ? 3 : 2 * n);

    bool fail = false;
    do {
        bool entry_done = false;
        if (!fd_entry(entry_done)) { fail = true; break; }
        if (!entry_done && !eval_f(B.x, xh, y)) { fail = true; break; }
        ++ret.fCalls;
        ++seq;
        if (!sumsq(y, 0)) { fail = true; break; }
        MIRLSQ_LAUNCH(k_init_state<T>, dim3(1), dim3(1), 0, stream, B.sum, B.st, st_slot_d[seq & 1], seq);
        if (!ok(hipGetLastError(), "init state") || !wait_state(seq)) { fail = true; break; }
    } while (false);
    if (fail) { teardown(); ret.status = mir_ls_numericError; return ret; }

    ret.residual = st_h->residual;
    bool fConverged = LM_F_CONVERGED(ret.residual, sd);
    bool needJacobian = true;
    bool last_rejected = false;
    bool spec_live = false;
    bool spec_predict = true;
    const bool speculate = device_cb && !no_speculation;
    uint32_t age = maxAge;
// ... 237 lines not shown
```

mir_optim_amd/csrc/unit_entries.hip:

```cpp
#include <cstddef>
#include <cstring>
#include <memory>
#include <vector>

#include "broyden_launch.h"
#include "driver.h"
#include "fit_spline_gpu.h"
#include "misc_kernels.h"

using namespace mirlsq;

namespace {
__global__ __launch_bounds__(256) void k_selftest_reductions(int rounds, uint32_t seed, int* out)
{
#pragma clang fp contract(off)
    uint32_t sr = seed ^ (0x9E3779B9u * (blockIdx.x * blockDim.x + threadIdx.x + 1));
    auto rnd = [&]() { sr ^= sr << 13; sr ^= sr >> 17; sr ^= sr << 5; return sr; };
    int bad[4] = {0, 0, 0, 0};
    for (int it = 0; it < rounds; ++it) {
        const float f = (float)(int32_t)rnd() * (1.0f / 65536.0f) * ((it & 7) == 0 ? 1e-20f : 1.0f);
        const double d = ((double)(int32_t)rnd() + (double)rnd() * 2.3283064365386963e-10) * ((it & 3) == 0 ? 1e-200 : 1.0);
        auto ref_sum = [](auto v) {
            v += __shfl_xor(v, 8, kWave); v += __shfl_xor(v, 4, kWave); v += __shfl_xor(v, 2, kWave); v += __shfl_xor(v, 1, kWave);
            v += __shfl_xor(v, 16, kWave); v += __shfl_xor(v, 32, kWave);
// ... 75 lines not shown
    };
    const size_t rJJ = take(nn, sizeof(T)), rJy = take(n, sizeof(T)), rx = take(n, sizeof(T)), rlo = take(n, sizeof(T)),
                 rup = take(n, sizeof(T)), rdx = take((size_t)kChainMax * n, sizeof(T)), rtr = take((size_t)kChainMax * n, sizeof(T)),
                 rrec = take(kChainMax, sizeof(ChainRec<T>)), rst = take(1, sizeof(LmState<T>));
    size_t rsc[kChainMax][7];
    for (int k = 0; k < kChainMax; ++k) {
        rsc[k][0] = take(nn, sizeof(T)); rsc[k][1] = take(nn, sizeof(T)); rsc[k][2] = take((size_t)n * (n | 1), sizeof(T));
        rsc[k][3] = take((size_t)12 * n, sizeof(T)); rsc[k][4] = take((size_t)2 * n, sizeof(int32_t));
        rsc[k][5] = take(n > kSolveMaxN ? kCoopWords : 0, sizeof(unsigned long long));
        rsc[k][6] = take(coop_scratch_elems(n), sizeof(T));
    }
    const size_t total = align_up(off + kLmGuardBytes, 256);
    char* base = nullptr;
    if (hipMalloc((void**)&base, total) != hipSuccess) return -3;
    auto at = [&](size_t r) { return base + reg[r].off; };
    LmSolveArgs<T> a{};
    a.JJ = (T*)at(rJJ); a.Jy = (T*)at(rJy); a.x = (T*)at(rx); a.lower = (T*)at(rlo); a.upper = (T*)at(rup);
    a.dx = (T*)at(rdx); a.trial = (T*)at(rtr); a.rec = (ChainRec<T>*)at(rrec); a.st = (LmState<T>*)at(rst);
    a.set = lm_settings_dev(settings); a.n = n;
    for (int k = 0; k < kChainMax; ++k) {
        a.sc[k].Pm = (T*)at(rsc[k][0]); a.sc[k].A = (T*)at(rsc[k][1]); a.sc[k].Fg = (T*)at(rsc[k][2]); a.sc[k].vec = (T*)at(rsc[k][3]);
        a.sc[k].ivec = (int32_t*)at(rsc[k][4]); a.sc[k].dbg = nullptr; a.sc[k].coop = (unsigned long long*)at(rsc[k][5]);
        a.sc[k].cS = (T*)at(rsc[k][6]);
        a.lam[k] = k < ks ? lam[k] : T(0);
    }
    a.f_in_lds = solve_nb(n, (int)sizeof(T)) > 0;
    a.check_grad = (mode & 1u) ? 1 : 0;
    a.lambda_from_state = (mode & 2u) ? 1 : 0;
    bool bounded = (mode & 4u) != 0;
    for (int i = 0; i < n; ++i)
        if (lower[i] > -Lim<T>::inf() || upper[i] < Lim<T>::inf()) bounded = true;
    const bool generic = (mode & 8u) != 0;
    a.coop_w = coop_width(n, query_num_cu(), !(mode & 16u));
    a.coop_epoch = a.coop_w > 1 ? 1u : 0u;
    const LmSolveClass cls = lm_solve_class((int)sizeof(T), n, bounded, generic, false);
    info[0] = cls.kind; info[1] = cls.nb; info[2] = cls.bounded; info[3] = a.coop_w; info[4] = -1; info[5] = (int)reg.size() + 1;

    LmState<T> st{};
    st.lambda = state_lambda;
    std::vector<T> sentinel((size_t)kChainMax * n, T(MIR_LSQ_LM_SOLVE_SENTINEL));
    bool good = hipMemset(base, 0xFF, total) == hipSuccess;
    auto up_ = [&](size_t r, const void* src) { good = good && hipMemcpy(at(r), src, reg[r].bytes, hipMemcpyHostToDevice) == hipSuccess; };
    up_(rJJ, JJ); up_(rJy, Jy); up_(rx, x); up_(rlo, lower); up_(rup, upper); up_(rdx, sentinel.data()); up_(rtr, sentinel.data());
    up_(rst, &st);
    for (int k = 0; k < kChainMax; ++k)
        if (reg[rsc[k][5]].bytes) good = good && hipMemset(at(rsc[k][5]), 0, reg[rsc[k][5]].bytes) == hipSuccess;
    if (!good) { (void)hipFree(base); return -3; }
    if (launch_lm_solve<T>(a, ks, bounded, generic, nullptr) != hipSuccess) { (void)hipDeviceSynchronize(); (void)hipFree(base); return -4; }
    std::unique_ptr<unsigned char[]> img(new unsigned char[total]);
    auto band = [&](size_t b, size_t& lo, size_t& hi) {
        lo = b ? reg[b - 1].off + reg[b - 1].bytes : 0; hi = b < reg.size() ? reg[b].off : total;
    };
    good = hipGetLastError() == hipSuccess && hipDeviceSynchronize() == hipSuccess
        && hipMemcpy(img.get(), base, reg[rsc[0][0]].off, hipMemcpyDeviceToHost) == hipSuccess;
    for (size_t b = rsc[0][0] + 1; b <= reg.size() && good; ++b) {
        size_t lo, hi;
        band(b, lo, hi);
        good = hipMemcpy(img.get() + lo, base + lo, hi - lo, hipMemcpyDeviceToHost) == hipSuccess;
    }
    (void)hipFree(base);
    if (!good) return -5;
    for (size_t b = 0; b <= reg.size() && info[4] < 0; ++b) {
        size_t lo, hi;
        band(b, lo, hi);
        for (size_t i = lo; i < hi; ++i)
            if (img[i] != 0xFF) { info[4] = (int)b; break; }
    }
    auto down = [&](size_t r, void* dst, size_t bytes) { std::memcpy(dst, img.get() + reg[r].off, bytes); };
    down(rJJ, JJ, reg[rJJ].bytes); down(rJy, Jy, reg[rJy].bytes); down(rx, x, reg[rx].bytes); down(rlo, lower, reg[rlo].bytes);
    down(rup, upper, reg[rup].bytes); down(rdx, dx, reg[rdx].bytes); down(rtr, trial, reg[rtr].bytes);
    std::vector<ChainRec<T>> rh(kChainMax);
    down(rrec, rh.data(), reg[rrec].bytes);
    for (int k = 0; k < ks; ++k) {
        rec[k].lambda = rh[k].lambda; rec[k].new_dx_dot = rh[k].new_dx_dot; rec[k].predicted = rh[k].predicted;
        rec[k].trial_xnorm = rh[k].trial_xnorm; rec[k].qp_status = rh[k].qp_status; rec[k].qp_iterations = rh[k].qp_iterations;
        rec[k].flags = rh[k].flags; rec[k].reserved = 0;
    }
    down(rst, &st, sizeof st);
    *jy_inf = st.jy_inf;
    return 0;
}

template <typename T, typename R>
int lr_pass_entry(size_t m, size_t n_, int k, const T* J, T* U, T* D, const T* dx, const T* dx_dot, const T* y, int count,
                  const T* y_old, T* JJ, T* Jy, const R* spec, T absTolerance, T relTolerance, T* partials, T* reduced, T* sums,
                  T* jy_inf, int info[6])
{
    if (!J || !U || !D || !dx || !dx_dot || !y || !y_old || !JJ || !Jy || !partials || !reduced || !sums || !jy_inf || !info) return -1;
    if (m == 0 || n_ == 0 || n_ > (size_t)kLrMaxN || k < 0 || k >= kLrMax || count < 1 || count > kChainMax) return -1;
    if (!device_available()) return -2;
    const int n = (int)n_, len = lr_len(n);
    const int nblk = lr_blocks(m, query_num_cu());
    struct Region { size_t off, bytes; };
    std::vector<Region> reg;
    size_t off = 0;
    auto take = [&](size_t cnt, size_t elem) {
        off = align_up(off + kLmGuardBytes, 256);
        reg.push_back({off, cnt * elem});
        off += cnt * elem;
        return reg.size() - 1;
    };
    const size_t rpart = take((size_t)nblk * len, sizeof(T)), rvec = take(len, sizeof(T)), rsp = take((size_t)count * nblk, sizeof(T)),
                 rsum = take(count, sizeof(T)), rst = take(1, sizeof(LmState<T>)), rrec = take(1, sizeof(ChainRec<T>));
    const size_t total = align_up(off + kLmGuardBytes, 256);
    char* base = nullptr;
    if (hipMalloc((void**)&base, total) != hipSuccess) return -3;
    auto at = [&](size_t r) { return base + reg[r].off; };
    const LrClass cls = lr_class_of<T>(n, J);
    info[0] = cls.ncp; info[1] = cls.vec; info[2] = nblk; info[3] = -1; info[4] = (int)reg.size() + 1; info[5] = 0;
    ChainRec<T> rec{};
    if (spec) {
        rec.lambda = spec->lambda; rec.new_dx_dot = spec->new_dx_dot; rec.predicted = spec->predicted; rec.trial_xnorm = spec->trial_xnorm;
        rec.qp_status = spec->qp_status; rec.qp_iterations = spec->qp_iterations; rec.flags = spec->flags; rec.pad = spec->reserved;
    }
    bool good = hipMemset(base, 0xFF, total) == hipSuccess;
    if (spec) good = good && hipMemcpy(at(rrec), &rec, sizeof rec, hipMemcpyHostToDevice) == hipSuccess;
    if (!good) { (void)hipFree(base); return -3; }
    LrArgs<T> a{};
    a.J = J; a.U = U; a.D = D; a.dx = dx; a.dx_dot = dx_dot; a.y = y; a.y_old = y_old;
    a.partials = (T*)at(rpart); a.m = m; a.n = n; a.k = k;
    a.spec_rec = spec ? (const ChainRec<T>*)at(rrec) : nullptr;
    a.absTolerance = absTolerance; a.relTolerance = relTolerance;
    good = lr_sweep<T>(a, nblk, nullptr) == hipSuccess
        && lr_reduce<T>((const T*)at(rpart), nblk, n, (T*)at(rvec), nullptr) == hipSuccess
        && (spec || lr_finish<T>((const T*)at(rvec), D, dx, k, n, JJ, Jy, (LmState<T>*)at(rst), nullptr) == hipSuccess)
        && lr_sumsq<T>(y, m, count, m, (T*)at(rsp), nblk, nblk, nullptr) == hipSuccess
        && lr_sumsq_final<T>((const T*)at(rsp), nblk, nblk, count, (T*)at(rsum), nullptr) == hipSuccess;
    if (!good) { (void)hipDeviceSynchronize(); (void)hipFree(base); return -4; }
    std::unique_ptr<unsigned char[]> img(new unsigned char[total]);
    good = hipGetLastError() == hipSuccess && hipDeviceSynchronize() == hipSuccess
        && hipMemcpy(img.get(), base, total, hipMemcpyDeviceToHost) == hipSuccess;
    (void)hipFree(base);
    if (!good) return -5;
    for (size_t b = 0; b <= reg.size() && info[3] < 0; ++b) {
        const size_t lo = b ? reg[b - 1].off + reg[b - 1].bytes : 0, hi = b < reg.size() ? reg[b].off : total;
        for (size_t i = lo; i < hi; ++i)
            if (img[i] != 0xFF) { info[3] = (int)b; break; }
    }
    const size_t jlo = offsetof(LmState<T>, jy_inf), jhi = jlo + sizeof(T);
    for (size_t i = 0; i < sizeof(LmState<T>); ++i)
        if ((i < jlo || i >= jhi || spec) && img[reg[rst].off + i] != 0xFF) info[5] |= 1;
    std::vector<unsigned char> want(sizeof rec, 0xFF);
    if (spec) std::memcpy(want.data(), &rec, sizeof rec);
    if (std::memcmp(img.get() + reg[rrec].off, want.data(), sizeof rec) != 0) info[5] |= 2;
    std::memcpy(partials, img.get() + reg[rpart].off, reg[rpart].bytes);
    std::memcpy(reduced, img.get() + reg[rvec].off, reg[rvec].bytes);
    std::memcpy(sums, img.get() + reg[rsum].off, reg[rsum].bytes);
    std::memcpy(jy_inf, img.get() + reg[rst].off + jlo, sizeof(T));
    return 0;
}

template <typename T>
int lr_flush_entry(size_t m, size_t n, int k, T* J, const T* U, const T* D, int info[2])
{
    if (!J || !U || !D || !info || m == 0 || n == 0 || n > (size_t)kLrMaxN || k < 1 || k > kLrMax) return -1;
    if (!device_available()) return -2;
    const LrClass cls = lr_class_of<T>((int)n, J);
    info[0] = cls.ncp; info[1] = cls.vec;
    if (lr_flush<T>(J, U, D, k, m, (int)n, query_num_cu(), nullptr) != hipSuccess) { (void)hipDeviceSynchronize(); return -4; }
    return hipGetLastError() == hipSuccess && hipDeviceSynchronize() == hipSuccess ? 0 : -5;
}

struct Banded {
    struct Region { size_t off, bytes; };
    std::vector<Region> reg;
    size_t off = 0, total = 0;
    bool pinned = false;
    char* base = nullptr;
    char* host = nullptr;
    std::unique_ptr<unsigned char[]> img;
    ~Banded() { if (pinned) { if (host) (void)hipHostFree(host); } else if (base) (void)hipFree(base); }
    size_t take(size_t count, size_t elem)
    {
        off = align_up(off + kLmGuardBytes, 256);
        reg.push_back({off, count * elem});
        off += count * elem;
        return reg.size() - 1;
    }
    bool alloc(bool pinned_ = false)
    {
        pinned = pinned_;
        total = align_up(off + kLmGuardBytes, 256);
        if (pinned) {
            if (hipHostMalloc((void**)&host, total, hipHostMallocMapped | hipHostMallocCoherent) != hipSuccess) { host = nullptr; return false; }
            std::memset(host, 0xFF, total);
            return hipHostGetDevicePointer((void**)&base, host, 0) == hipSuccess;
        }
        if (hipMalloc((void**)&base, total) != hipSuccess) { base = nullptr; return false; }
        return hipMemset(base, 0xFF, total) == hipSuccess;
    }
    char* at(size_t r) const { return base + reg[r].off; }
    bool up(size_t r, const void* src, size_t bytes) const
    {
        if (bytes > reg[r].bytes) return false;
        if (!bytes) return true;
        if (pinned) { std::memcpy(host + reg[r].off, src, bytes); return true; }
        return hipMemcpy(at(r), src, bytes, hipMemcpyHostToDevice) == hipSuccess;
    }
    bool up(size_t r, const void* src) const { return up(r, src, reg[r].bytes); }
    bool fetch()
    {
        img.reset(new unsigned char[total]);
        if (pinned) { std::memcpy(img.get(), host, total); return true; }
        return hipMemcpy(img.get(), base, total, hipMemcpyDeviceToHost) == hipSuccess;
    }
    int damaged() const
// ... 207 lines not shown
    if (hipMalloc((void**)&packed, sizeof(double) * packed_len) != hipSuccess) { (void)hipFree(slabs); return -3; }
    if (hipMalloc((void**)&st, sizeof(LmState<double>)) != hipSuccess) { (void)hipFree(slabs); (void)hipFree(packed); return -3; }
    int rc = 0;
    JtjArgs<double> a{};
    a.J = Yrm; a.Jout = J; a.y = y; a.y_old = y; a.dx = nullptr; a.dx_dot = nullptr; a.slabs = slabs; a.m = m; a.n = (int)n;
    a.twh = twh;
    hipEvent_t e0, e1;
    (void)hipEventCreate(&e0); (void)hipEventCreate(&e1);
    (void)hipEventRecord(e0, stream);
    if (jtj_run<double>(plan, op, a, packed, stream) != hipSuccess) rc = -4;
    (void)hipEventRecord(e1, stream);
    (void)jtj_unpack<double>(packed, (int)n, JJ, Jy, st, stream);
    if (hipStreamSynchronize(stream) != hipSuccess) rc = -5;
    if (kernel_ms) { float ms = 0; (void)hipEventElapsedTime(&ms, e0, e1); *kernel_ms = ms; }
    (void)hipEventDestroy(e0); (void)hipEventDestroy(e1);
    (void)hipFree(slabs); (void)hipFree(packed); (void)hipFree(st);
    return rc;
}
}

extern "C" {

int mir_solve_box_qp_gpu_d(const mir_box_qp_settings_d* settings, size_t n, const double* P, const double* q,
                           const double* l, const double* u, double* x, int unconstrainedSolution, int* iterations)
{
    return box_qp_entry<double>(settings, n, P, q, l, u, x, unconstrainedSolution, iterations);
}
int mir_solve_box_qp_gpu_s(const mir_box_qp_settings_s* settings, size_t n, const float* P, const float* q,
                           const float* l, const float* u, float* x, int unconstrainedSolution, int* iterations)
{
    return box_qp_entry<float>(settings, n, P, q, l, u, x, unconstrainedSolution, iterations);
}

int mir_lsq_jtj_d(size_t m, size_t n, double* J, const double* y, const double* y_old, const double* dx, int broyden,
                  double* JJ, double* Jy, void* stream, float* kernel_ms)
{
    return jtj_entry<double>(m, n, J, y, y_old, dx, broyden, JJ, Jy, stream, kernel_ms);
}
int mir_lsq_fd_jtj_d(size_t m, size_t n, const double* Yrm, const double* twh, const double* y, double* J,
                     double* JJ, double* Jy, void* stream_, float* kernel_ms)
{
    return fd_jtj_entry(m, n, Yrm, twh, y, J, JJ, Jy, stream_, kernel_ms, false);
}
int mir_lsq_fd_diff_jtj_d(size_t m, size_t n, const double* Drm, const double* twh, const double* y, double* J,
                          double* JJ, double* Jy, void* stream_, float* kernel_ms)
{
    return fd_jtj_entry(m, n, Drm, twh, y, J, JJ, Jy, stream_, kernel_ms, true);
}
int mir_lsq_jtj_plan(size_t elem_size, size_t m, size_t n, int num_cu, int op, int aligned16, size_t out[10])
{
    if ((elem_size != 4 && elem_size != 8) || m == 0 || n == 0 || n > (size_t)1 << 20 || num_cu < 1 || op < 0 || op > 3 || !out) return -1;
    const JtjPlan p = elem_size == 8 ? jtj_plan<double>(m, (int)n, num_cu) : jtj_plan<float>(m, (int)n, num_cu);
    const JtjLaunch l = jtj_resolve(p, (JtjOp)op, aligned16 != 0);
    const bool wide = l.kernel == JtjKernel::wide;
    const size_t v[10] = {(size_t)l.kernel, (size_t)l.ncb, (size_t)l.flat, (size_t)l.nblk, (size_t)l.njobs, l.lds,
                          (size_t)l.nblk * l.njobs, (size_t)l.slab_len, wide ? 0 : (size_t)l.ncb, jtj_slab_elems(p)};
    for (int i = 0; i < 10; ++i) out[i] = v[i];
    return 0;
}
int mir_lsq_lm_solve_d(const mir_least_squares_settings_d* settings, size_t n, double* JJ, double* Jy, double* x, double* lower,
                       double* upper, int ks, const double* lam, double state_lambda, unsigned mode, mir_lsq_lm_solve_record_d* rec,
                       double* dx, double* trial, double* jy_inf, int info[6])
{
    return lm_solve_entry<double>(settings, n, JJ, Jy, x, lower, upper, ks, lam, state_lambda, mode, rec, dx, trial, jy_inf, info);
}
int mir_lsq_lm_solve_s(const mir_least_squares_settings_s* settings, size_t n, float* JJ, float* Jy, float* x, float* lower,
                       float* upper, int ks, const float* lam, float state_lambda, unsigned mode, mir_lsq_lm_solve_record_s* rec,
                       float* dx, float* trial, float* jy_inf, int info[6])
{
    return lm_solve_entry<float>(settings, n, JJ, Jy, x, lower, upper, ks, lam, state_lambda, mode, rec, dx, trial, jy_inf, info);
}
int mir_lsq_lm_solve_class(size_t elem_size, size_t n, int bounded, int generic, int diagnostic, int out[3])
{
    if ((elem_size != 4 && elem_size != 8) || n == 0 || n > (size_t)1 << 20 || !out) return -1;
    const LmSolveClass c = lm_solve_class((int)elem_size, (int)n, bounded != 0, generic != 0, diagnostic != 0);
    out[0] = c.kind; out[1] = c.nb; out[2] = c.bounded;
    return 0;
}
int mir_lsq_lr_pass_d(size_t m, size_t n, int k, const double* J, double* U, double* D, const double* dx, const double* dx_dot,
                      const double* y, int count, const double* y_old, double* JJ, double* Jy, const mir_lsq_lm_solve_record_d* spec,
                      double absTolerance, double relTolerance, double* partials, double* reduced, double* sums, double* jy_inf,
                      int info[6])
{
    return lr_pass_entry<double>(m, n, k, J, U, D, dx, dx_dot, y, count, y_old, JJ, Jy, spec, absTolerance, relTolerance, partials,
                                 reduced, sums, jy_inf, info);
}
int mir_lsq_lr_pass_s(size_t m, size_t n, int k, const float* J, float* U, float* D, const float* dx, const float* dx_dot,
                      const float* y, int count, const float* y_old, float* JJ, float* Jy, const mir_lsq_lm_solve_record_s* spec,
                      float absTolerance, float relTolerance, float* partials, float* reduced, float* sums, float* jy_inf,
                      int info[6])
{
    return lr_pass_entry<float>(m, n, k, J, U, D, dx, dx_dot, y, count, y_old, JJ, Jy, spec, absTolerance, relTolerance, partials,
                                reduced, sums, jy_inf, info);
}
int mir_lsq_lr_flush_d(size_t m, size_t n, int k, double* J, const double* U, const double* D, int info[2])
{
    return lr_flush_entry<double>(m, n, k, J, U, D, info);
}
int mir_lsq_lr_flush_s(size_t m, size_t n, int k, float* J, const float* U, const float* D, int info[2])
{
    return lr_flush_entry<float>(m, n, k, J, U, D, info);
}
int mir_lsq_lr_class(size_t elem_size, size_t n, int aligned, int out[2])
{
    if ((elem_size != 4 && elem_size != 8) || n == 0 || n > (size_t)kLrMaxN || !out) return -1;
    const LrClass c = lr_class((int)n, aligned != 0);
    out[0] = c.ncp; out[1] = c.vec;
    return 0;
}
int mir_lsq_lr_blocks(size_t m, int num_cu)
{
    if (m == 0) return -1;
    if (num_cu <= 0) {
        if (!device_available()) return -2;
        num_cu = query_num_cu();
    }
    return lr_blocks(m, num_cu);
}
int mir_lsq_decide_d(const mir_least_squares_settings_d* settings, size_t n, int ks, unsigned mode, uint32_t maxIterations, uint32_t seq,
                     mir_lsq_lm_state_d* state, mir_lsq_lm_solve_record_d* rec, double* sums, double* x, double* trial, double* dx_chain,
                     double* dx_acc, double* partials, int nparts, int pstride, mir_lsq_lm_state_d* host_state, double* host_x, int info[2])
{
    return decide_entry<double>(settings, n, ks, mode, maxIterations, seq, state, rec, sums, x, trial, dx_chain, dx_acc, partials, nparts,
                                pstride, host_state, host_x, info);
}
int mir_lsq_decide_s(const mir_least_squares_settings_s* settings, size_t n, int ks, unsigned mode, uint32_t maxIterations, uint32_t seq,
                     mir_lsq_lm_state_s* state, mir_lsq_lm_solve_record_s* rec, float* sums, float* x, float* trial, float* dx_chain,
                     float* dx_acc, float* partials, int nparts, int pstride, mir_lsq_lm_state_s* host_state, float* host_x, int info[2])
{
    return decide_entry<float>(settings, n, ks, mode, maxIterations, seq, state, rec, sums, x, trial, dx_chain, dx_acc, partials, nparts,
                               pstride, host_state, host_x, info);
}
int mir_lsq_fd_points_d(size_t n, const double* x, const double* lower, const double* upper, double eps, int with_base, double* X,
                        double* twh, double* twh_host, int info[2])
{
    return fd_points_entry<double>(n, x, lower, upper, eps, with_base, X, twh, twh_host, info);
}
int mir_lsq_fd_points_s(size_t n, const float* x, const float* lower, const float* upper, float eps, int with_base, float* X,
                        float* twh, float* twh_host, int info[2])
{
    return fd_points_entry<float>(n, x, lower, upper, eps, with_base, X, twh, twh_host, info);
}
int mir_lsq_fd_fill_d(size_t m, size_t n, size_t ldy, int j0, int pc, const double* Y, const double* twh, double* J, int col, int info[2])
{
    return fd_fill_entry<double>(m, n, ldy, j0, pc, Y, twh, J, col, info);
}
int mir_lsq_fd_fill_s(size_t m, size_t n, size_t ldy, int j0, int pc, const float* Y, const float* twh, float* J, int col, int info[2])
{
    return fd_fill_entry<float>(m, n, ldy, j0, pc, Y, twh, J, col, info);
}
int mir_lsq_entry_state_d(size_t m, const double* v, uint32_t seq, double* partials, double* sum, mir_lsq_lm_state_d* state,
                          mir_lsq_lm_state_d* host_state, double* partials2, double* sums2, mir_lsq_lm_state_d* st2, int info[3])
{
    return entry_state_entry<double>(m, v, seq, partials, sum, state, host_state, partials2, sums2, st2, info);
}
int mir_lsq_entry_state_s(size_t m, const float* v, uint32_t seq, float* partials, float* sum, mir_lsq_lm_state_s* state,
                          mir_lsq_lm_state_s* host_state, float* partials2, float* sums2, mir_lsq_lm_state_s* st2, int info[3])
{
    return entry_state_entry<float>(m, v, seq, partials, sum, state, host_state, partials2, sums2, st2, info);
}
int mir_lsq_sumsq_blocks(size_t m) { return m ? sumsq_blocks(m) : -1; }
int mir_lsq_unpack_grad_d(size_t n, const double* packed, mir_lsq_lm_state_d* state, double* JJ, double* Jy, int info[2])
{
    return unpack_grad_entry<double>(n, packed, state, JJ, Jy, info);
}
int mir_lsq_unpack_grad_s(size_t n, const float* packed, mir_lsq_lm_state_s* state, float* JJ, float* Jy, int info[2])
{
    return unpack_grad_entry<float>(n, packed, state, JJ, Jy, info);
}
int mir_lsq_jtj_s(size_t m, size_t n, float* J, const float* y, const float* y_old, const float* dx, int broyden,
                  float* JJ, float* Jy, void* stream, float* kernel_ms)
{
    return jtj_entry<float>(m, n, J, y, y_old, dx, broyden, JJ, Jy, stream, kernel_ms);
}
int mir_lsq_selftest_reductions(int rounds, int mismatches[4])
{
// ... 39 lines not shown
```

Baseline: 1181.

## Skip writing FD Jacobian; Broyden sweep reads scaled difference panel directly

When the finite-difference Jacobian is built from the difference panel and low-rank Broyden updates are active, the fused FD+JtJ kernel no longer writes J to memory. The Broyden low-rank sweep and flush instead read the raw difference panel and scale each element by the inverse step width on the fly, from LDS or registers. This removes one full m×n write of J per full Jacobian evaluation. In exchange it adds per-element scaling work and extra shared-memory traffic in the sweep, and the flush must later materialise J from the panel. It applies only to f64 with n ≤ 256.

```diff
diff --git a/include/mir_optim_amd.h b/include/mir_optim_amd.h
--- a/include/mir_optim_amd.h
+++ b/include/mir_optim_amd.h
@@ -135,6 +135,7 @@
     MIR_LSQ_VARIANT_SOLVE_GENERIC = 1u << 10,
     MIR_LSQ_VARIANT_SOLVE_ONE_WORKGROUP = 1u << 11,
     MIR_LSQ_VARIANT_NO_FD_BASE_POINT = 1u << 14,
+    MIR_LSQ_VARIANT_FD_WRITE_J = 1u << 15,
     MIR_LSQ_VARIANT_FD_HOST_COLUMNS = 1u << 13,
     MIR_LSQ_VARIANT_NO_PIPELINE = 1u << 22,
     MIR_LSQ_VARIANT_DEBUG_HELPERS_ABSENT = 1u << 12,
@@ -413,6 +414,12 @@
                       int info[6]);
 int mir_lsq_lr_flush_d(size_t m, size_t n, int k, double* J, const double* U, const double* D, int info[2]);
 int mir_lsq_lr_flush_s(size_t m, size_t n, int k, float* J, const float* U, const float* D, int info[2]);
+int mir_lsq_lr_pass_scaled_d(size_t m, size_t n, int k, const double* P, const double* twh, double* U, double* D, const double* dx,
+                             const double* dx_dot, const double* y, int count, const double* y_old, double* JJ, double* Jy,
+                             const mir_lsq_lm_solve_record_d* spec, double absTolerance, double relTolerance, double* partials,
+                             double* reduced, double* sums, double* jy_inf, int info[6]);
+int mir_lsq_lr_flush_scaled_d(size_t m, size_t n, int k, double* J, const double* P, const double* twh, const double* U, const double* D,
+                              int info[2]);
 int mir_lsq_lr_class(size_t elem_size, size_t n, int aligned, int out[2]);
 int mir_lsq_lr_blocks(size_t m, int num_cu);
 
diff --git a/mir_optim_amd/api.py b/mir_optim_amd/api.py
--- a/mir_optim_amd/api.py
+++ b/mir_optim_amd/api.py
@@ -18,7 +18,7 @@
     "fit_spline_residuals", "variant_lr_cap",
     "VARIANT_BROYDEN_REWRITE", "VARIANT_FD_SEPARATE_FILL", "VARIANT_NO_SPECULATION", "VARIANT_NO_NULL_SKIP",
     "VARIANT_SOLVE_BOUNDED", "VARIANT_DEBUG_SOLVE", "VARIANT_HOST_PROFILE", "VARIANT_SOLVE_GENERIC", "VARIANT_SOLVE_ONE_WORKGROUP", "VARIANT_DEBUG_HELPERS_ABSENT", "VARIANT_FD_HOST_COLUMNS",
-    "VARIANT_NO_PIPELINE", "FD_BASE_POINT", "VARIANT_NO_FD_BASE_POINT", "BatchedOptions", "BatchedExtras", "BATCHED_ABSOLUTE_SIGMA", "BATCHED_BOUNDS_PER_PROBLEM",
+    "VARIANT_NO_PIPELINE", "FD_BASE_POINT", "VARIANT_NO_FD_BASE_POINT", "VARIANT_FD_WRITE_J", "BatchedOptions", "BatchedExtras", "BATCHED_ABSOLUTE_SIGMA", "BATCHED_BOUNDS_PER_PROBLEM",
     "covariance", "spdInverse", "COVARIANCE_ABSOLUTE_SIGMA",
     "fitSplineGpu", "splineEvalGpu", "fit_spline_eval_gpu", "fit_spline_eval_host", "fit_spline_factor",
     "lmSolve", "lm_solve_class",
@@ -49,6 +49,7 @@
 VARIANT_DEBUG_HELPERS_ABSENT = 1 << 12
 VARIANT_FD_HOST_COLUMNS = 1 << 13
 VARIANT_NO_FD_BASE_POINT = 1 << 14
+VARIANT_FD_WRITE_J = 1 << 15
 VARIANT_NO_PIPELINE = 1 << 22
 
 
@@ -311,6 +312,11 @@
             fn = getattr(L, "mir_lsq_lr_flush_" + suf)
             fn.restype = C.c_int
             fn.argtypes = [sz, sz, C.c_int, C.c_void_p, C.c_void_p, C.c_void_p, C.POINTER(C.c_int * 2)]
+        L.mir_lsq_lr_pass_scaled_d.restype = C.c_int
+        L.mir_lsq_lr_pass_scaled_d.argtypes = [sz, sz, C.c_int] + [C.c_void_p] * 7 + [C.c_int] + [C.c_void_p] * 4 \
+            + [C.c_double, C.c_double] + [C.c_void_p] * 4 + [C.POINTER(C.c_int * 6)]
+        L.mir_lsq_lr_flush_scaled_d.restype = C.c_int
+        L.mir_lsq_lr_flush_scaled_d.argtypes = [sz, sz, C.c_int] + [C.c_void_p] * 5 + [C.POINTER(C.c_int * 2)]
         L.mir_lsq_lr_class.restype = C.c_int
         L.mir_lsq_lr_class.argtypes = [sz, sz, C.c_int, C.POINTER(C.c_int * 2)]
         L.mir_lsq_lr_blocks.restype = C.c_int
@@ -960,8 +966,11 @@
     return rc
 
 
-def lrPass(m, n, k, J, U, D, dx, dx_dot, y, y_old, JJ, Jy, dtype=np.float64, count=1, spec=None, absTolerance=0.0, relTolerance=0.0):
+def lrPass(m, n, k, J, U, D, dx, dx_dot, y, y_old, JJ, Jy, dtype=np.float64, count=1, spec=None, absTolerance=0.0, relTolerance=0.0,
+           twh=None):
     dtype = np.dtype(dtype)
+    if twh is not None and dtype != np.float64:
+        raise ValueError("the scaled sweep exists in f64 only")
     nblk, ln = lr_blocks(m), lr_len(n)
     partials, reduced = np.zeros((nblk, ln), dtype=dtype), np.zeros(ln, dtype=dtype)
     sums, jy_inf = np.zeros(count, dtype=dtype), np.zeros(1, dtype=dtype)
@@ -971,10 +980,14 @@
         for key, v in spec.items():
             rec[key] = v
     info = (C.c_int * 6)()
-    fn = lib().mir_lsq_lr_pass_d if dtype == np.float64 else lib().mir_lsq_lr_pass_s
-    rc = fn(m, n, k, J, U, D, dx, dx_dot, y, count, y_old, JJ, Jy, rec.ctypes.data if rec is not None else None,
+    tail = (dx, dx_dot, y, count, y_old, JJ, Jy, rec.ctypes.data if rec is not None else None,
             float(absTolerance), float(relTolerance), partials.ctypes.data, reduced.ctypes.data, sums.ctypes.data, jy_inf.ctypes.data,
             C.byref(info))
+    if twh is not None:
+        rc = lib().mir_lsq_lr_pass_scaled_d(m, n, k, J, twh, U, D, *tail)
+    else:
+        fn = lib().mir_lsq_lr_pass_d if dtype == np.float64 else lib().mir_lsq_lr_pass_s
+        rc = fn(m, n, k, J, U, D, *tail)
     if rc != 0:
         raise RuntimeError(f"mir_lsq_lr_pass failed: {rc}")
     if info[2] != nblk:
@@ -989,6 +1002,14 @@
     rc = fn(m, n, k, J, U, D, C.byref(info))
     if rc != 0:
         raise RuntimeError(f"mir_lsq_lr_flush failed: {rc}")
+    return int(info[0]), bool(info[1])
+
+
+def lrFlushScaled(m, n, k, J, P, twh, U, D):
+    info = (C.c_int * 2)()
+    rc = lib().mir_lsq_lr_flush_scaled_d(m, n, k, J, P, twh, U, D, C.byref(info))
+    if rc != 0:
+        raise RuntimeError(f"mir_lsq_lr_flush_scaled failed: {rc}")
     return int(info[0]), bool(info[1])
 
 
@@ -1225,7 +1246,9 @@
     return d
 
 
-def fd_jtj(Yrm, twh, y, diff=False):
+def fd_jtj(Yrm, twh, y, diff=False, write_J=True):
+    if not write_J and not diff:
+        raise ValueError("only the difference-panel kernel takes a NULL J")
     L = lib()
     Yrm = np.ascontiguousarray(Yrm, dtype=np.float64)
     m, n2 = Yrm.shape
@@ -1237,10 +1260,10 @@
     dJJ = DeviceBuffer(nbytes=n * n * 8, dtype=np.float64, shape=(n, n))
     dJy = DeviceBuffer(nbytes=n * 8, dtype=np.float64, shape=(n,))
     ms = C.c_float(0)
-    rc = (L.mir_lsq_fd_diff_jtj_d if diff else L.mir_lsq_fd_jtj_d)(m, n, dY.ptr, dt.ptr, dy.ptr, dJ.ptr, dJJ.ptr, dJy.ptr, None, C.byref(ms))
+    rc = (L.mir_lsq_fd_diff_jtj_d if diff else L.mir_lsq_fd_jtj_d)(m, n, dY.ptr, dt.ptr, dy.ptr, dJ.ptr if write_J else None, dJJ.ptr, dJy.ptr, None, C.byref(ms))
     if rc != 0:
         raise RuntimeError(f"mir_lsq_fd_jtj_d failed: {rc}")
-    out = dJ.download(), dJJ.download(), dJy.download(), ms.value
+    out = dJ.download() if write_J else None, dJJ.download(), dJy.download(), ms.value
     for b in (dY, dt, dy, dJ, dJJ, dJy):
         b.free()
     return out
diff --git a/mir_optim_amd/csrc/broyden_launch.h b/mir_optim_amd/csrc/broyden_launch.h
--- a/mir_optim_amd/csrc/broyden_launch.h
+++ b/mir_optim_amd/csrc/broyden_launch.h
@@ -21,6 +21,7 @@
     const ChainRec<T>* spec_rec;
     T absTolerance, relTolerance;
 };
+constexpr int kLrScaledMaxN = 256;
 
 constexpr int kLrMaxBlocks = 1024;
 inline int lr_blocks(size_t m, int num_cu)
@@ -46,11 +47,13 @@
     return lr_class(n, reinterpret_cast<uintptr_t>(J) % (2 * sizeof(T)) == 0);
 }
 
-template <typename T> hipError_t lr_sweep(const LrArgs<T>& a, int nblk, hipStream_t s);
+template <typename T> hipError_t lr_sweep(const LrArgs<T>& a, int nblk, hipStream_t s, const T* twh = nullptr);
 template <typename T> hipError_t lr_reduce(const T* partials, int nblk, int n, T* out, hipStream_t s);
 template <typename T> hipError_t lr_finish(const T* lr, T* D, const T* dx, int k, int n, T* JJ, T* Jy, LmState<T>* st, hipStream_t s);
 template <typename T> hipError_t lr_sumsq(const T* v, size_t m, int count, size_t vstride, T* partials, int pstride, int nblk, hipStream_t s);
 template <typename T> hipError_t lr_sumsq_final(const T* partials, int pstride, int nblk, int count, T* out, hipStream_t s);
 template <typename T> hipError_t lr_flush(T* J, const T* U, const T* D, int k, size_t m, int n, int num_cu, hipStream_t s);
+hipError_t lr_flush_scaled(double* J, const double* P, const double* twh, const double* U, const double* D, int k, size_t m, int n,
+                           int num_cu, hipStream_t s);
 
 }
diff --git a/mir_optim_amd/csrc/broyden_lr.h b/mir_optim_amd/csrc/broyden_lr.h
--- a/mir_optim_amd/csrc/broyden_lr.h
+++ b/mir_optim_amd/csrc/broyden_lr.h
@@ -41,9 +41,12 @@
     return yy;
 }
 
-template <typename T, int NCP, bool VEC>
-__global__ __launch_bounds__(256, (NCP <= 4 ? 4 : 1)) void k_broyden_lr(const LrArgs<T> a)
-{
+template <typename A> __device__ __forceinline__ A lr_only(A a) { return a; }
+template <typename T, int NCP, bool VEC, typename... Src>
+__global__ __launch_bounds__(256, (NCP <= 4 ? 4 : 1)) void k_broyden_lr(const LrArgs<T> a, const Src... src)
+{
+    constexpr bool SCALED = sizeof...(Src) == 1;
+    static_assert(sizeof...(Src) <= 1, "at most the widths");
     using P2 = typename LrPair<T>::type;
     __shared__ T red[4][lr_len(kLrMaxN)];
     __shared__ T coef[kLrMax];
@@ -85,6 +88,22 @@
         d0[c] = ok0[c] ? t0 : T(0);
         d1[c] = ok1[c] ? t1 : T(0);
     }
+    constexpr bool INV_LDS = SCALED && !VEC;
+    T* const invt = &red[0][0];
+    T* const dxt = invt + kLrScaledMaxN;
+    T i0[SCALED && !INV_LDS ? NCP : 1], i1[SCALED && !INV_LDS ? NCP : 1];
+    if constexpr (INV_LDS) {
+        const T* __restrict__ twh = lr_only(src...);
+        for (int j = threadIdx.x; j < n; j += blockDim.x) invt[j] = fd_inv_width(twh[j]);
+        for (int j = threadIdx.x; j < 32 * NCP; j += blockDim.x) dxt[j] = j < n ? a.dx[j] : T(0);
+    } else if constexpr (SCALED) {
+        const T* __restrict__ twh = lr_only(src...);
+#pragma unroll
+        for (int c = 0; c < NCP; ++c) {
+            i0[c] = fd_inv_width(twh[coff[c]]);
+            i1[c] = fd_inv_width(twh[coff[c] + 1]);
+        }
+    }
     __syncthreads();
     const bool own = p < k;
     const T cp = own ? coef[p] : T(0);
@@ -125,13 +144,36 @@
 #pragma unroll
         for (int e = 0; e < UNR; ++e) {
             if (g0 + e < ge) {
+                [[maybe_unused]] int lo = 0;
+                if constexpr (INV_LDS) { lo = 2 * p; asm volatile("" : "+v"(lo)); }
+                if constexpr (SCALED) {
+#pragma unroll
+                    for (int c = 0; c < NCP; ++c) {
+                        if constexpr (INV_LDS) {
+                            v0[e][c] = fd_scale(v0[e][c], invt[ok0[c] ? 32 * c + lo : 0]);
+                            v1[e][c] = fd_scale(v1[e][c], invt[ok1[c] ? 32 * c + lo + 1 : 0]);
+                            d0[c] = dxt[32 * c + lo];
+                            d1[c] = dxt[32 * c + lo + 1];
+                        } else {
+                            v0[e][c] = fd_scale(v0[e][c], i0[c]);
+                            v1[e][c] = fd_scale(v1[e][c], i1[c]);
+                        }
+                    }
+                }
                 const size_t row = 4 * (g0 + e) + q;
                 const bool rok = row < m;
                 T yn = ynv[e];
                 const T yo = yov[e], ul = ulv[e];
                 T s = ul * cp;
-#pragma unroll
-                for (int c = 0; c < NCP; ++c) s += v0[e][c] * d0[c] + v1[e][c] * d1[c];
+                if constexpr (SCALED) {
+#pragma clang fp contract(off)
+                    s = dfma(ul, cp, dfma(v0[e][0], d0[0], v1[e][0] * d1[0]));
+#pragma unroll
+                    for (int c = 1; c < NCP; ++c) s = s + dfma(v0[e][c], d0[c], v1[e][c] * d1[c]);
+                } else {
+#pragma unroll
+                    for (int c = 0; c < NCP; ++c) s += v0[e][c] * d0[c] + v1[e][c] * d1[c];
+                }
                 s = sum16(s);
                 T u = nd * ((yo - yn) + s);
                 if (!rok) { u = 0; yn = 0; }
@@ -152,6 +194,7 @@
         }
     }
 
+    if constexpr (INV_LDS) __syncthreads();
     auto qsum = [](T v) { v += wave_shfl_xor(v, 16); v += wave_shfl_xor(v, 32); return v; };
 #pragma unroll
     for (int c = 0; c < NCP; ++c) { va0[c] = qsum(va0[c]); va1[c] = qsum(va1[c]); ga0[c] = qsum(ga0[c]); ga1[c] = qsum(ga1[c]); }
@@ -281,10 +324,13 @@
     }
 }
 
-template <typename T, int NCP, bool VEC>
+template <typename T> struct LrFlushSrc { const T* P; const T* twh; };
+template <typename T, int NCP, bool VEC, typename... Src>
 __global__ __launch_bounds__(256) void k_lr_flush(T* J, const T* __restrict__ U, const T* __restrict__ D,
-                                                  int k, size_t m, int n)
-{
+                                                  int k, size_t m, int n, const Src... src)
+{
+    constexpr bool SCALED = sizeof...(Src) == 1;
+    static_assert(sizeof...(Src) <= 1, "at most the panel and its widths");
     using P2 = typename LrPair<T>::type;
     extern __shared__ unsigned char lr_smem[];
     T* Ds = reinterpret_cast<T*>(lr_smem);
@@ -300,6 +346,14 @@
         ok0[c] = col < n;
         ok1[c] = col + 1 < n;
         coff[c] = ok0[c] ? col : 0;
+    }
+    T i0[SCALED ? NCP : 1], i1[SCALED ? NCP : 1];
+    if constexpr (SCALED) {
+#pragma unroll
+        for (int c = 0; c < NCP; ++c) {
+            i0[c] = fd_inv_width(lr_only(src...).twh[coff[c]]);
+            i1[c] = fd_inv_width(lr_only(src...).twh[(VEC || ok1[c]) ? coff[c] + 1 : 0]);
+        }
     }
     const size_t G = (m + 3) / 4;
     const size_t wave_id = ((size_t)blockIdx.x * blockDim.x + threadIdx.x) >> 6;
@@ -310,6 +364,7 @@
         const size_t rr = rok ? row : m - 1;
         T* rp = J + rr * (size_t)n;
         const T* sp = rp;
+        if constexpr (SCALED) sp = lr_only(src...).P + rr * (size_t)n;
         T v0[NCP], v1[NCP];
 #pragma unroll
         for (int c = 0; c < NCP; ++c) {
@@ -322,6 +377,7 @@
                 v0[c] = sp[coff[c]];
                 v1[c] = sp[ok1[c] ? coff[c] + 1 : 0];
             }
+            if constexpr (SCALED) { v0[c] = fd_scale(v0[c], i0[c]); v1[c] = fd_scale(v1[c], i1[c]); }
         }
         for (int l = 0; l < k; ++l) {
             const T ul = U[(size_t)l * m + rr];
diff --git a/mir_optim_amd/csrc/common.h b/mir_optim_amd/csrc/common.h
--- a/mir_optim_amd/csrc/common.h
+++ b/mir_optim_amd/csrc/common.h
@@ -27,6 +27,10 @@
 
 __device__ inline double dfma(double a, double b, double c) { return __builtin_fma(a, b, c); }
 __device__ inline float dfma(float a, float b, float c) { return __builtin_fmaf(a, b, c); }
+__device__ __forceinline__ double fd_inv_width(double t) { return t == 0 ? 0.0 : 1.0 / t; }
+__device__ __forceinline__ double fd_scale(double d, double inv) { return inv == 0 ? 0.0 : d * inv; }
+__device__ __forceinline__ double fd_jacobian_element(double d, double t) { return fd_scale(d, fd_inv_width(t)); }
+
 constexpr int kLrMax = 16;
 __host__ __device__ constexpr int lr_len(int n) { return 2 * n + 2 * kLrMax + 3; }
 __host__ __device__ constexpr int lr_yy(int n) { return 2 * n + 2 * kLrMax + 2; }
diff --git a/mir_optim_amd/csrc/driver.h b/mir_optim_amd/csrc/driver.h
--- a/mir_optim_amd/csrc/driver.h
+++ b/mir_optim_amd/csrc/driver.h
@@ -148,6 +148,9 @@
     FB fbr = nullptr;
     FB fbd = nullptr;
     int fd_fused = 0;
+    bool j0_in_panel = false;
+    const T* lr_j0() const { return j0_in_panel ? static_cast<const T*>(ws->ypanel) : B.J; }
+    const T* lr_twh() const { return j0_in_panel ? B.twh : nullptr; }
     bool fd_base_point = false;
     bool fd_entry_ready = false;
     size_t fd_entry_event = (size_t)-1;
diff --git a/mir_optim_amd/csrc/launch_broyden.hip b/mir_optim_amd/csrc/launch_broyden.hip
--- a/mir_optim_amd/csrc/launch_broyden.hip
+++ b/mir_optim_amd/csrc/launch_broyden.hip
@@ -27,9 +27,25 @@
 }
 }
 template <typename T>
-hipError_t lr_sweep(const LrArgs<T>& a, int nblk, hipStream_t s)
+hipError_t lr_sweep(const LrArgs<T>& a, int nblk, hipStream_t s, const T* twh)
 {
     if (a.n > kLrMaxN || a.k < 0 || a.k >= kLrMax) return hipErrorInvalidValue;
+    if (twh) {
+        if constexpr (std::is_same<T, double>::value) {
+            if (a.n > kLrScaledMaxN) return hipErrorInvalidValue;
+            return lr_dispatch(lr_class_of<T>(a.n, a.J), [&](auto ncp, auto vec) {
+                constexpr int NCP = decltype(ncp)::value;
+                if constexpr (NCP <= kLrScaledMaxN / 32) {
+                    MIRLSQ_LAUNCH((k_broyden_lr<T, NCP, decltype(vec)::value, const T*>), dim3(nblk), dim3(256), 0, s, a, twh);
+                    return hipGetLastError();
+                } else {
+                    return hipErrorInvalidValue;
+                }
+            });
+        } else {
+            return hipErrorInvalidValue;
+        }
+    }
     return lr_dispatch(lr_class_of<T>(a.n, a.J), [&](auto ncp, auto vec) {
         MIRLSQ_LAUNCH((k_broyden_lr<T, decltype(ncp)::value, decltype(vec)::value>), dim3(nblk), dim3(256), 0, s, a);
         return hipGetLastError();
@@ -49,6 +65,28 @@
     return lr_dispatch(lr_class_of<T>(n, J), [&](auto ncp, auto vec) {
         MIRLSQ_LAUNCH((k_lr_flush<T, decltype(ncp)::value, decltype(vec)::value>), dim3((unsigned)blocks), dim3(256), lds, s, J, U, D, k, m, n);
         return hipGetLastError();
+    });
+}
+
+hipError_t lr_flush_scaled(double* J, const double* P, const double* twh, const double* U, const double* D, int k, size_t m, int n,
+                           int num_cu, hipStream_t s)
+{
+    if (n > kLrScaledMaxN || k < 0 || k > kLrMax || !P || !twh) return hipErrorInvalidValue;
+    const size_t G = (m + 3) / 4;
+    size_t blocks = (G + 3) / 4;
+    if (blocks > (size_t)num_cu * 8) blocks = (size_t)num_cu * 8;
+    if (blocks < 1) blocks = 1;
+    const size_t lds = (size_t)k * n * sizeof(double);
+    const bool aligned = reinterpret_cast<uintptr_t>(J) % 16 == 0 && reinterpret_cast<uintptr_t>(P) % 16 == 0;
+    return lr_dispatch(lr_class(n, aligned), [&](auto ncp, auto vec) {
+        constexpr int NCP = decltype(ncp)::value;
+        if constexpr (NCP <= kLrScaledMaxN / 32) {
+            MIRLSQ_LAUNCH((k_lr_flush<double, NCP, decltype(vec)::value, LrFlushSrc<double>>), dim3((unsigned)blocks), dim3(256), lds, s, J, U, D, k, m, n,
+                          LrFlushSrc<double>{P, twh});
+            return hipGetLastError();
+        } else {
+            return hipErrorInvalidValue;
+        }
     });
 }
 
@@ -82,7 +120,7 @@
 }
 
 #define MIRLSQ_INSTANTIATE(T)                                                                                             \
-    template hipError_t lr_sweep<T>(const LrArgs<T>&, int, hipStream_t);                                                  \
+    template hipError_t lr_sweep<T>(const LrArgs<T>&, int, hipStream_t, const T*);                                        \
     template hipError_t lr_reduce<T>(const T*, int, int, T*, hipStream_t);                                                \
     template hipError_t lr_finish<T>(const T*, T*, const T*, int, int, T*, T*, LmState<T>*, hipStream_t);                 \
     template hipError_t lr_sumsq<T>(const T*, size_t, int, size_t, T*, int, int, hipStream_t);                            \
diff --git a/mir_optim_amd/csrc/solver_jacobian.hip b/mir_optim_amd/csrc/solver_jacobian.hip
--- a/mir_optim_amd/csrc/solver_jacobian.hip
+++ b/mir_optim_amd/csrc/solver_jacobian.hip
@@ -1,3 +1,5 @@
+#include <type_traits>
+
 #include "driver.h"
 #include "launch_util.h"
 #include "misc_kernels.h"
@@ -11,18 +13,25 @@
     if (lr_k >= lr_cap) {
         const uint64_t launches_before = launches_now();
         struct Excl { Solver* s; uint64_t l0; ~Excl() { s->launches_excluded += s->launches_now() - l0; } } excl{this, launches_before};
-        if (!ok(lr_flush<T>(B.J, U, B.lrD, lr_k, m, (int)n, ws->num_cu, stream), "broyden flush")) return false;
+        if (j0_in_panel) {
+            if constexpr (std::is_same<T, double>::value) {
+                if (!ok(lr_flush_scaled(B.J, lr_j0(), B.twh, U, B.lrD, lr_k, m, (int)n, ws->num_cu, stream), "broyden flush")) return false;
+            } else {
+                return false;
+            }
+            j0_in_panel = false;
+        } else if (!ok(lr_flush<T>(B.J, U, B.lrD, lr_k, m, (int)n, ws->num_cu, stream), "broyden flush")) return false;
         lr_k = 0;
         if (stats) stats->broyden_flushes++;
         if (!plain_products(yold_dev)) return false;
         if (stats) stats->jtj_resyncs++;
     }
     LrArgs<T> a{};
-    a.J = B.J; a.U = U; a.D = B.lrD; a.dx = B.dx_acc; a.dx_dot = &B.st->dx_dot; a.y = y_dev; a.y_old = yold_dev;
+    a.J = lr_j0(); a.U = U; a.D = B.lrD; a.dx = B.dx_acc; a.dx_dot = &B.st->dx_dot; a.y = y_dev; a.y_old = yold_dev;
     a.partials = B.lrpart; a.m = m; a.n = (int)n; a.k = lr_k;
     const int nblk = lr_blocks(m, ws->num_cu), len = lr_len((int)n);
     ev_begin(1);
-    if (!ok(lr_sweep<T>(a, nblk, stream), "broyden sweep")) return false;
+    if (!ok(lr_sweep<T>(a, nblk, stream, lr_twh()), "broyden sweep")) return false;
     ev_end();
     if (!ok(lr_reduce<T>(B.lrpart, nblk, (int)n, B.lrvec, stream), "broyden reduce")) return false;
     if (comm && !allreduce(B.lrvec, (size_t)len, 1)) return false;
@@ -57,7 +66,7 @@
 bool Solver<T>::jacobian_products(bool broyden, const T* y_dev, const T* yold_dev)
 {
     if (broyden && lowrank) return broyden_lowrank(y_dev, yold_dev);
-    if (!broyden) lr_k = 0;
+    if (!broyden) { lr_k = 0; j0_in_panel = false; }
     JtjArgs<T> a{};
     a.J = B.J; a.Jout = B.J; a.y = y_dev; a.y_old = yold_dev; a.dx = B.dx_acc; a.dx_dot = &B.st->dx_dot;
     a.slabs = B.slabs; a.m = m; a.n = (int)n;
@@ -65,6 +74,10 @@
         const JtjOp op = fd_fused == 2 ? JtjOp::fd_diff : JtjOp::fd;
         fd_fused = 0;
         a.J = static_cast<const T*>(ws->ypanel); a.twh = B.twh;
+        if (op == JtjOp::fd_diff && lowrank && n <= (uint32_t)kLrScaledMaxN && !(variant & MIR_LSQ_VARIANT_FD_WRITE_J)) {
+            j0_in_panel = true;
+            a.Jout = nullptr;
+        }
         const bool direct = unpack_in_reduce(op);
         ev_begin(3);
         if (!ok(jtj_run<T>(plan, op, a, B.packed, stream, direct ? unpack_target() : JtjUnpack<T>{}), "fd + jtj kernel")) return false;
diff --git a/mir_optim_amd/csrc/solver_loop.hip b/mir_optim_amd/csrc/solver_loop.hip
--- a/mir_optim_amd/csrc/solver_loop.hip
+++ b/mir_optim_amd/csrc/solver_loop.hip
@@ -318,13 +318,13 @@
     spec_events_from = events.size();
     if (stats) stats->fused_rounds++;
     LrArgs<T> a{};
-    a.J = B.J; a.U = static_cast<T*>(ws->ulr); a.D = B.lrD; a.dx = B.dx; a.dx_dot = &B.rec[0].new_dx_dot; a.y = ytr; a.y_old = y;
+    a.J = lr_j0(); a.U = static_cast<T*>(ws->ulr); a.D = B.lrD; a.dx = B.dx; a.dx_dot = &B.rec[0].new_dx_dot; a.y = ytr; a.y_old = y;
     a.partials = B.lrpart; a.m = m; a.n = (int)n; a.k = lr_k;
     a.spec_rec = B.rec; a.absTolerance = sd.absTolerance; a.relTolerance = sd.relTolerance;
     const int nblk = lr_blocks(m, ws->num_cu), len = lr_len((int)n);
     spec_enqueue = true;
     ev_begin(1);
-    const bool swept = ok(lr_sweep<T>(a, nblk, stream), "broyden sweep");
+    const bool swept = ok(lr_sweep<T>(a, nblk, stream, lr_twh()), "broyden sweep");
     ev_end();
     spec_enqueue = false;
     if (!swept || !ok(lr_reduce<T>(B.lrpart, nblk, (int)n, B.lrvec, stream), "broyden reduce")) return false;
diff --git a/mir_optim_amd/csrc/unit_entries.hip b/mir_optim_amd/csrc/unit_entries.hip
--- a/mir_optim_amd/csrc/unit_entries.hip
+++ b/mir_optim_amd/csrc/unit_entries.hip
@@ -181,7 +181,7 @@
 }
 
 template <typename T, typename R>
-int lr_pass_entry(size_t m, size_t n_, int k, const T* J, T* U, T* D, const T* dx, const T* dx_dot, const T* y, int count,
+int lr_pass_entry(size_t m, size_t n_, int k, const T* J, const T* twh, T* U, T* D, const T* dx, const T* dx_dot, const T* y, int count,
                   const T* y_old, T* JJ, T* Jy, const R* spec, T absTolerance, T relTolerance, T* partials, T* reduced, T* sums,
                   T* jy_inf, int info[6])
 {
@@ -220,7 +220,7 @@
     a.partials = (T*)at(rpart); a.m = m; a.n = n; a.k = k;
     a.spec_rec = spec ? (const ChainRec<T>*)at(rrec) : nullptr;
     a.absTolerance = absTolerance; a.relTolerance = relTolerance;
-    good = lr_sweep<T>(a, nblk, nullptr) == hipSuccess
+    good = lr_sweep<T>(a, nblk, nullptr, twh) == hipSuccess
         && lr_reduce<T>((const T*)at(rpart), nblk, n, (T*)at(rvec), nullptr) == hipSuccess
         && (spec || lr_finish<T>((const T*)at(rvec), D, dx, k, n, JJ, Jy, (LmState<T>*)at(rst), nullptr) == hipSuccess)
         && lr_sumsq<T>(y, m, count, m, (T*)at(rsp), nblk, nblk, nullptr) == hipSuccess
@@ -594,7 +594,7 @@
                       double absTolerance, double relTolerance, double* partials, double* reduced, double* sums, double* jy_inf,
                       int info[6])
 {
-    return lr_pass_entry<double>(m, n, k, J, U, D, dx, dx_dot, y, count, y_old, JJ, Jy, spec, absTolerance, relTolerance, partials,
+    return lr_pass_entry<double>(m, n, k, J, nullptr, U, D, dx, dx_dot, y, count, y_old, JJ, Jy, spec, absTolerance, relTolerance, partials,
                                  reduced, sums, jy_inf, info);
 }
 int mir_lsq_lr_pass_s(size_t m, size_t n, int k, const float* J, float* U, float* D, const float* dx, const float* dx_dot,
@@ -602,8 +602,27 @@
                       float absTolerance, float relTolerance, float* partials, float* reduced, float* sums, float* jy_inf,
                       int info[6])
 {
-    return lr_pass_entry<float>(m, n, k, J, U, D, dx, dx_dot, y, count, y_old, JJ, Jy, spec, absTolerance, relTolerance, partials,
+    return lr_pass_entry<float>(m, n, k, J, nullptr, U, D, dx, dx_dot, y, count, y_old, JJ, Jy, spec, absTolerance, relTolerance, partials,
                                 reduced, sums, jy_inf, info);
+}
+int mir_lsq_lr_pass_scaled_d(size_t m, size_t n, int k, const double* P, const double* twh, double* U, double* D, const double* dx,
+                             const double* dx_dot, const double* y, int count, const double* y_old, double* JJ, double* Jy,
+                             const mir_lsq_lm_solve_record_d* spec, double absTolerance, double relTolerance, double* partials,
+                             double* reduced, double* sums, double* jy_inf, int info[6])
+{
+    if (!twh || n > (size_t)kLrScaledMaxN) return -1;
+    return lr_pass_entry<double>(m, n, k, P, twh, U, D, dx, dx_dot, y, count, y_old, JJ, Jy, spec, absTolerance, relTolerance, partials,
+                                 reduced, sums, jy_inf, info);
+}
+int mir_lsq_lr_flush_scaled_d(size_t m, size_t n, int k, double* J, const double* P, const double* twh, const double* U, const double* D,
+                              int info[2])
+{
+    if (!J || !P || !twh || !U || !D || !info || m == 0 || n == 0 || n > (size_t)kLrScaledMaxN || k < 1 || k > kLrMax) return -1;
+    if (!device_available()) return -2;
+    const LrClass cls = lr_class((int)n, reinterpret_cast<uintptr_t>(J) % 16 == 0 && reinterpret_cast<uintptr_t>(P) % 16 == 0);
+    info[0] = cls.ncp; info[1] = cls.vec;
+    if (lr_flush_scaled(J, P, twh, U, D, k, m, (int)n, query_num_cu(), nullptr) != hipSuccess) { (void)hipDeviceSynchronize(); return -4; }
+    return hipGetLastError() == hipSuccess && hipDeviceSynchronize() == hipSuccess ? 0 : -5;
 }
 int mir_lsq_lr_flush_d(size_t m, size_t n, int k, double* J, const double* U, const double* D, int info[2])
 {
```

Result: faster. 1208, median of 6 (+2.3%).
